# Createroner/InSAR-Unet-CA

Hardware: AMD Instinct MI355X
Metric: InSAR tiles/sec (fwd+bwd) U-Net-CA 256x256 (higher is better)
Workload: dtype bf16; 1 GPU; U-Net-CA (in=2, classes=2, use_se) bf16, batch 16x2x256x256 per GPU, Dice+CE + Adam(lr=1e-4) training on synthetic InSAR tiles; global_batch=16, parallelism=dp1

## Files before the change

### include/insar_hip.h

```cpp
#ifndef INSAR_HIP_H
#define INSAR_HIP_H

#include <stdint.h>

#ifdef __cplusplus
extern "C" {
#endif

#define INSAR_ABI_VERSION 8

enum { INSAR_F32 = 0, INSAR_BF16 = 1 };

enum {
  INSAR_OK = 0,
  INSAR_E_SHAPE = -1001,
  INSAR_E_DTYPE = -1002,
  INSAR_E_ALIGN = -1003,
  INSAR_E_WS = -1004,
  INSAR_E_ARG = -1005
};

typedef struct InsarAct {
  void* ptr;
  int32_t B, H, W;
// ... 27 lines not shown

typedef struct InsarIgemm {
  InsarAct x;
  InsarAct y;
  const void* w;
  const float* bias;
  float* stats;
  int32_t N;
  int32_t Ho, Wo;
  int32_t stride;
  int32_t ntaps;
  int32_t mode;
  int8_t dy[12], dx[12];
  int32_t flags;
  int32_t out_stride;
  int32_t out_oy, out_ox;
  int32_t _pad;
  const void* add;
  InsarBstat bstat;
  const void* gate;
} InsarIgemm;
enum { INSAR_IGEMM_OOB_ZERO = 1,
       INSAR_IGEMM_PINGPONG = 2  };
int insar_igemm_num_mtiles(int64_t M, int32_t N);
int insar_igemm_tile_rows(int64_t M, int32_t N);
int insar_igemm_tile_cols(int64_t M, int32_t N);
int insar_igemm_tile_cols_dt(int64_t M, int32_t N, int32_t dtype);
int insar_igemm(const InsarIgemm* d, void* stream);

int insar_conv3x3_flat_ok(const InsarAct* x, int32_t N);
int insar_conv3x3_flat_num_mtiles(const InsarAct* x);
int insar_conv3x3_flat_rows_ok(const InsarAct* x, int32_t N);
int insar_conv3x3_flat_rows_dil_ok(const InsarAct* x, int32_t N, int32_t dil);
int insar_conv3x3_flat2_rows_ok(const InsarAct* x, int32_t N);
int insar_conv3x3_flat_stat_rows(const InsarAct* x, int32_t N, int32_t flip);
int insar_conv3x3_flat(const InsarAct* x, const InsarAct* y, const void* w, int32_t flip, float* stats,
                       void* stream);
int insar_conv3x3_flat_bstat(const InsarAct* x, const InsarAct* y, const void* w, int32_t flip, float* stats,
                             const InsarBstat* bstat, void* stream);

int insar_conv3x3_c64_ok(const InsarAct* x, int32_t N);
int insar_conv3x3_c64_rows(const InsarAct* x);
int insar_conv3x3_c64_geometry(const InsarAct* x, int32_t* out);
int insar_conv3x3_c64(const InsarAct* x, const InsarAct* y, const void* w, int32_t flip, float* stats,
                      void* stream);
int insar_conv3x3_c64_bstat(const InsarAct* x, const InsarAct* y, const void* w, int32_t flip, float* stats,
                            const InsarBstat* bstat, void* stream);

typedef struct InsarWgrad {
  InsarAct x;
  InsarAct dy;
  const int32_t* tabx;
  const int32_t* tabdy;
  float* part;
  int64_t Mpad;
  int32_t nsplit;
  int32_t ntaps;
  int32_t offx[12];
  int32_t offdy[12];
  int64_t tabx_tap_stride;
} InsarWgrad;
int insar_wgrad_tile(int32_t C, int32_t dtype);
int insar_wgrad_tile_pair(int32_t Cin, int32_t Cout, int32_t dtype);
int insar_wgrad(const InsarWgrad* d, void* stream);
int insar_wgrad_conv3_tile(const InsarAct* x, int32_t Cout);
int insar_wgrad_conv3(const InsarAct* x, const InsarAct* dy, float* part, int32_t nsplit, void* stream);
int insar_wgrad_conv3x_tile(const InsarAct* x, int32_t Cout);
int insar_wgrad_conv3x(const InsarAct* x, const InsarAct* dy, float* part, int32_t nsplit, void* stream);
int insar_wgrad_conv3y_tile(const InsarAct* x, int32_t Cout);
int insar_wgrad_conv3y(const InsarAct* x, const InsarAct* dy, float* part, int32_t nsplit, void* stream);
int insar_wgrad_conv3k_tile(const InsarAct* x, int32_t Cout);
int insar_wgrad_conv3k_slices(const InsarAct* x, int32_t Cout);
int insar_wgrad_conv3k(const InsarAct* x, const InsarAct* dy, float* part, int32_t nsplit, void* stream);
int insar_wgrad_reduce(const float* part, float* grad, int32_t nsplit, int32_t ntaps, int32_t Co,
                       int32_t Ci, int32_t layout, int32_t accumulate, void* stream);
int insar_wgrad_fold(const float* part_in, float* part_out, int64_t slab_floats, int32_t nsplit,
                     int32_t group, void* stream);
int insar_pixel_table(int32_t* tab, int64_t Mpad, int32_t B, int32_t H, int32_t W, int32_t s,
                      int32_t Hb, int32_t Wb, int32_t tail, void* stream);

int insar_conv3x3_small_fwd_rows(const InsarAct* x, const InsarAct* y);
int insar_conv3x3_small_fwd(const InsarAct* x, const float* w ,
                            const InsarAct* y, float* stats , void* stream);
int insar_conv3x3_small_wgrad_blocks(int32_t B, int32_t H);
int insar_conv3x3_small_wgrad(const InsarAct* x, const InsarAct* dy, float* part, void* stream);
int insar_conv3x3_small_wgrad_fused_ok(const InsarAct* x, const InsarAct* y);
int insar_conv3x3_small_wgrad_fused(const InsarAct* x, const InsarAct* g, const InsarAct* y, const float* scale,
                                    const float* shift, const float* mean, const float* invstd, const float* k1,
                                    const float* k2, int32_t relu, float* part, void* stream);

int insar_colsum(const float* part, float* out, int32_t segments, int64_t rows, int32_t cols,
                 int32_t accumulate, float* tmp, int64_t tmp_floats, void* stream);
int insar_colsum_ld(const float* part, float* out, int32_t segments, int64_t rows, int32_t cols, int64_t ld,
                    int32_t accumulate, float* tmp, int64_t tmp_floats, void* stream);

int insar_colsum_partial(const float* part, float* out, int64_t rows, int32_t cols, int32_t rps,
                         void* stream);

typedef struct InsarBnFinalize {
  const float* part; int64_t rows; int64_t count; int32_t C; int32_t training;
  const float* conv_bias; const float* gamma; const float* beta;
  float* running_mean; float* running_var; int64_t* num_batches_tracked;
  float momentum; float eps;
  float* scale; float* shift; float* mean; float* invstd;
} InsarBnFinalize;
int insar_bn_finalize(const InsarBnFinalize* d, void* stream);
int insar_bn_relu_apply(const InsarAct* y, const float* scale, const float* shift,
                        const float* gate , const InsarAct* dst, int32_t relu,
                        void* stream);

int insar_bn_relu_apply_pool(const InsarAct* y, const float* scale, const float* shift, const float* gate,
                             const InsarAct* dst, const InsarAct* pooled, int32_t relu, void* stream);

int insar_se_squeeze(const InsarAct* y, const float* scale, const float* shift, float* part,
                     int32_t relu, int32_t rows_per_part, void* stream);
typedef struct InsarSeFwd {
  const float* part;
  int32_t B, H, W, C, Cr; int32_t rows;
  const float* scale; const float* shift;
  const float* w1;  const float* w2;
  float* pooled;
  float* sq; float* hid; float* gate;
} InsarSeFwd;
int insar_se_excite(const InsarSeFwd* d, void* stream);

int insar_bnrelu_bwd_reduce(const InsarAct* dout, const InsarAct* y, const float* scale,
                            const float* shift, float* part, int32_t relu, int32_t rows_per_part, void* stream);
typedef struct InsarBnSeBwd {
  int32_t B, H, W, C, Cr; int32_t use_se;
  const float* mean; const float* invstd;
  const float* pooled; const float* sq; const float* hid; const float* gate;
  const float* w1; const float* w2;
  float* dw1; float* dw2; float* dgamma; float* dbeta;
  float* coefB; float* k1; float* k2;
  int32_t accumulate; int32_t _pad;
} InsarBnSeBwd;
int insar_bnse_bwd_coef(const InsarBnSeBwd* d, const float* red, int32_t rows, const float* scale,
                        const float* shift, float* ws, float* dconv_bias, int32_t training, void* stream);
int insar_bnse_bwd_coef_fused(const InsarBnSeBwd* d, const float* red, int32_t rows, const float* scale,
                              const float* shift, float* ws, float* dconv_bias, int32_t training, uint32_t* ticket,
                              void* stream);
int insar_bn_bwd_coef(const InsarBnSeBwd* d, const float* red, int64_t rows_total, const float* scale,
                      float* dconv_bias, int32_t training, void* stream);
int insar_bnrelu_bwd_apply(const InsarAct* dout, const InsarAct* y, const float* scale,
                           const float* shift, const float* mean, const float* invstd,
                           const float* gate, const float* coefB, const float* k1,
                           const float* k2, const InsarAct* dy, int32_t relu, void* stream);
int insar_bnse_bwd_coef_stage(const InsarBnSeBwd* d, const float* red, int32_t rows, const float* scale,
                              const float* shift, float* ws, float* dconv_bias, int32_t training, int32_t stage,
                              void* stream);
int insar_bnrelu_bwd_apply_part(const InsarAct* dout, const InsarAct* y, const float* scale, const float* shift,
                                const float* mean, const float* invstd, const float* gate, const float* coefB,
                                const float* tb, const float* tg, const InsarAct* dy, int32_t relu, void* stream);

int insar_bn_relu_apply_pool_arg(const InsarAct* y, const float* scale, const float* shift, const float* gate,
                                 const InsarAct* dst, const InsarAct* pooled, uint8_t* arg, int32_t relu, void* stream);
int insar_bnrelu_bwd_reduce_pool(const InsarAct* dskip, const InsarAct* dpooled, const uint8_t* arg, const InsarAct* y,
                                 const float* scale, const float* shift, float* part, int32_t relu,
                                 int32_t rows_per_part, void* stream);
int insar_bnrelu_bwd_apply_pool(const InsarAct* dskip, const InsarAct* dpooled, const uint8_t* arg, const InsarAct* y,
                                const float* scale, const float* shift, const float* mean, const float* invstd,
                                const float* gate, const float* coefB, const float* k1, const float* k2,
                                const InsarAct* dy, int32_t relu, void* stream);

int insar_conv1x1_out_wgrad(const InsarAct* x, const float* w, const float* dlogits, int32_t K, float* part, void* stream);
int insar_bn_relu_apply_outc(const InsarAct* y, const float* scale, const float* shift, const float* gate ,
                             const float* wout, const float* bias , float* logits, int32_t K, int32_t relu,
                             void* stream);
int insar_conv1x1_out_wgrad_y(const InsarAct* y, const float* scale, const float* shift, const float* gate ,
                              const float* w, const float* dlogits, int32_t K, float* part, void* stream);
int insar_bnrelu_bwd_reduce_outc(const float* dlogits, const float* wout, int32_t K, const InsarAct* y,
                                 const float* scale, const float* shift, float* part, int32_t relu,
                                 int32_t rows_per_part, const float* gate, float* wpart, void* stream);
int insar_bnrelu_bwd_apply_outc(const float* dlogits, const float* wout, int32_t K, const InsarAct* y,
                                const float* scale, const float* shift, const float* mean, const float* invstd,
                                const float* gate, const float* coefB, const float* k1, const float* k2,
                                const InsarAct* dy, int32_t relu, void* stream);

typedef struct InsarCam {
  int32_t B, H, W, C, Cr; int32_t rows;
  const float* psum; const float* pmax; const int32_t* parg;
  const float* w1; const float* w2;
  float* avg; float* mx; int32_t* arg;
  float* ha; float* hm;
  float* gate;
  float* coefB; float* dmax;
  float* ws;
  float* dw1; float* dw2;
  int32_t accumulate; int32_t _pad;
} InsarCam;
int insar_cam_pool(const InsarAct* x, float* psum, float* pmax, int32_t* parg, int32_t rows_per_part,
                   void* stream);
int insar_cam_excite(const InsarCam* d, void* stream);
int insar_cam_bwd_coef(const InsarCam* d, const float* red , int32_t rows, void* stream);
int insar_cam_scatter_max(const InsarAct* dx, const float* dmax, const int32_t* arg, void* stream);

typedef struct InsarSa {
  InsarAct x;
  InsarAct y;
  float* comp;
  uint16_t* arg;
  float* z1; float* z2;
  float* s;
  float* g2; float* g1;
  float* dcomp;
  float* stat1; float* stat2;
  float* part;
  int32_t rows;
  int32_t training;
  const float* w1; const float* w2;
  const float* bn;
  float* coef;
  float* dw1; float* db1; float* dgamma1; float* dbeta1;
  float* dw2; float* db2; float* dgamma2; float* dbeta2;
} InsarSa;
int insar_sa_compress(const InsarSa* d, void* stream);
int insar_sa_conv(const InsarSa* d, int32_t which , void* stream);
int insar_sa_gate(const InsarSa* d, void* stream);
int insar_sa_dscale(const InsarSa* d, void* stream);
int insar_sa_bwd_coef(const InsarSa* d, int32_t stage , void* stream);
int insar_sa_bwd_stencil(const InsarSa* d, int32_t which , void* stream);
int insar_sa_dx(const InsarSa* d, void* stream);

int insar_maxpool2_fwd(const InsarAct* x, const InsarAct* y, void* stream);
int insar_maxpool2_bwd(const InsarAct* x, const InsarAct* dy, const InsarAct* dx, int32_t accumulate,
                       void* stream);

int insar_resize_bilinear_fwd(const InsarAct* src, const InsarAct* dst, void* stream);
int insar_resize_bilinear_bwd(const InsarAct* ddst, const InsarAct* dsrc, void* stream);

int insar_conv1x1_out_fwd(const InsarAct* x, const float* w , const float* bias,
                          float* logits , int32_t K, void* stream);
int insar_conv1x1_out_bwd_blocks(int32_t B, int32_t H);
int insar_conv1x1_out_bwd(const InsarAct* x, const float* w, const float* dlogits, int32_t K,
                          const InsarAct* dx, float* part, void* stream);

int insar_ce_blocks(int64_t npix);
int insar_cross_entropy(const float* logits, const int64_t* target, int32_t B, int32_t K, int64_t HW,
                        int64_t ignore_index, float* dlogits, float* loss_out, float* ws, void* stream);
int insar_dice(const float* logits, const int64_t* target, int32_t B, int32_t K, int64_t HW,
               int64_t ignore_index, float smooth, float* dlogits, float* loss_out, float* ws,
               void* stream);

int insar_dice_ce(const float* logits, const int64_t* target, int32_t B, int32_t K, int64_t HW,
                  int64_t ignore_index, float smooth, float ce_weight, float dice_weight, float* dlogits,
                  float* loss_out, float* ws, void* stream);

int insar_cross_entropy_w(const float* logits, const int64_t* target, int32_t B, int32_t K, int64_t HW,
                          int64_t ignore_index, const float* weight, float label_smoothing, float* dlogits,
                          float* loss_out, float* ws, void* stream);
int insar_focal(const float* logits, const int64_t* target, int32_t B, int32_t K, int64_t HW, int64_t ignore_index,
                float gamma, const float* alpha, float* dlogits, float* loss_out, float* ws, void* stream);
int insar_dice_ce_w(const float* logits, const int64_t* target, int32_t B, int32_t K, int64_t HW,
                    int64_t ignore_index, float smooth, float ce_weight, float dice_weight, const float* weight,
                    float label_smoothing, float focal_gamma, float* dlogits, float* loss_out, float* ws,
                    void* stream);
int insar_label_hist(const int64_t* target, int64_t npix, int32_t K, int64_t ignore_index, int64_t* counts,
                     int64_t* ws, void* stream);

int insar_confusion(const float* logits, const int64_t* target, int32_t B, int32_t K, int64_t HW,
                    int64_t ignore_index, int64_t* counts , void* stream);

enum { INSAR_SCENE_U8 = 0, INSAR_SCENE_F32 = 1 };
int insar_scene_gather(const void* scene, int32_t dtype , int32_t H, int32_t W, const int32_t* origins,
                       int32_t n, int32_t T, float* out , void* stream);
int insar_scene_blend(const float* logits, const int32_t* origins, int32_t n, int32_t K, int32_t T, int32_t overlap,
                      float* acc, float* wsum, int32_t H, int32_t W, int32_t y_lo, int32_t y_hi, int32_t x_lo, int32_t x_hi,
                      void* stream);
int insar_scene_finalize(const float* acc, const float* wsum, int32_t K, int32_t H, int32_t W, float* prob ,
                         uint8_t* mask, float* conf, void* stream);

typedef struct InsarRegion {
  int64_t area;
  int64_t sum_y, sum_x;
  int64_t sum_conf;
  int32_t y0, x0, y1, x1;
  int32_t root;
  int32_t cls;
  int32_t _pad[2];
} InsarRegion;
int insar_regions_scratch_bytes(int32_t H, int32_t W, int32_t max_regions, int64_t* scratch_bytes, int64_t* table_bytes);
int insar_regions_tiles(const uint8_t* mask, const float* conf , float min_conf, int32_t H, int32_t W,
                        int32_t connectivity, void* scratch, void* stream);
int insar_regions_merge(const uint8_t* mask, int32_t H, int32_t W, int32_t connectivity, void* scratch, void* stream);
int insar_regions_flatten(int32_t H, int32_t W, void* scratch, void* stream);
int insar_regions_number(const uint8_t* mask, int32_t H, int32_t W, int64_t min_area, int32_t max_regions, void* scratch,
                         void* table, void* stream);
int insar_regions_relabel(const uint8_t* mask, const float* conf , int32_t H, int32_t W, int32_t max_regions,
                          void* scratch, void* table, int32_t* labels, uint8_t* mask_out, void* stream);

typedef struct InsarOverlap {
  int32_t pred, gt;
  int64_t count;
} InsarOverlap;
int insar_overlap_scratch_bytes(int64_t max_pairs, int64_t* table_bytes, int64_t* out_bytes);
int insar_overlap_clear(void* table, void* out, int64_t max_pairs, void* stream);
int insar_overlap_count(const int32_t* pred, const int32_t* gt, const uint8_t* voidmap , int32_t void_value,
                        int32_t H, int32_t W, void* table, int64_t max_pairs, void* stream);
int insar_overlap_compact(const void* table, int64_t max_pairs, void* out, void* stream);

enum { INSAR_DIST_U8 = 0, INSAR_DIST_I32 = 1 };
enum { INSAR_DIST_EQ = 0, INSAR_DIST_NE = 1, INSAR_DIST_EDGE = 2 };
#define INSAR_DIST_FAR 0x7fffffff
int insar_dist_scratch_bytes(int32_t B, int32_t H, int32_t W, int64_t* scratch_bytes);
int insar_dist_transform(const void* m, int32_t elem_type, int32_t B, int32_t H, int32_t W, int32_t site_mode, int32_t value,
                         int32_t max_distance, void* scratch, int32_t* d2, int32_t* nearest , void* stream);
int insar_dist_boundary_counts(const uint8_t* pred, const uint8_t* gt, const int32_t* d2_pred, const int32_t* d2_gt, int32_t H,
                               int32_t W, int64_t r2, int32_t K, int32_t void_value, int64_t* counts, void* stream);

enum { INSAR_AUG_MASK_NONE = 0, INSAR_AUG_MASK_U8 = 1, INSAR_AUG_MASK_I64 = 2 };
int insar_aug_draw(uint64_t seed, uint64_t step, int32_t n, int32_t ops_mask, float gain_lo, float gain_hi, float bias_lo,
                   float bias_hi, float sigma_lo, float sigma_hi, int32_t* table, void* stream);
int insar_aug_apply(const float* x, float* xo, int32_t C, const void* m, int32_t m_dtype , int64_t* mo,
                    int32_t n, int32_t H, int32_t W, const int32_t* table, uint64_t noise_seed, void* stream);

int insar_crops_cells(const uint8_t* labels, int32_t H, int32_t W, int32_t K, int32_t g, int32_t* table, void* stream);
int insar_crops_sat(int32_t* table, int32_t K, int32_t Hc, int32_t Wc, void* stream);
int insar_crops_draw(uint64_t key, int32_t n, int32_t K, int32_t tries, const float* cum, int32_t min_count, int32_t max_void,
                     int32_t T, int32_t g, int32_t H, int32_t W, const int32_t* sat, int32_t* origins, int32_t* info, void* stream);
int insar_crops_gather(const void* scene, int32_t scene_dtype, const uint8_t* labels, int32_t H, int32_t W, const int32_t* origins,
                       int32_t n, int32_t T, float* images, void* masks, int32_t mask_dtype, void* stream);

int insar_adam_step(const int64_t* table, const int32_t* chunks, int32_t nchunks, int32_t chunk_elems,
                    float lr, float beta1, float beta2, float eps, float bias_correction1,
                    float bias_correction2_sqrt, float grad_scale, void* stream);

int insar_pixel_table_taps(int32_t* tab , int64_t Mpad, int32_t B, int32_t H, int32_t W, int32_t s,
                           int32_t Hb, int32_t Wb, int32_t ntaps, const int8_t* dy, const int8_t* dx, void* stream);
int insar_conv7x7s2_fwd_rows(int32_t B, int32_t H);
// ... 65 lines not shown
```

### insar_unet_ca_amd/_lib.py

```python
from __future__ import annotations

import ctypes as C
import os

import torch

_HERE = os.path.dirname(os.path.abspath(__file__))
LIB_PATH = os.environ.get("INSAR_HIP_LIB") or os.path.join(_HERE, "libinsar_hip.so")

F32, BF16 = 0, 1
ABI_VERSION = 8
SCENE_U8, SCENE_F32 = 0, 1
AUG_MASK_NONE, AUG_MASK_U8, AUG_MASK_I64 = 0, 1, 2
DIST_U8, DIST_I32 = 0, 1
DIST_EQ, DIST_NE, DIST_EDGE = 0, 1, 2
DIST_FAR = 0x7FFFFFFF
IGEMM_OOB_ZERO = 1
IGEMM_PINGPONG = 2


class InsarAct(C.Structure):
    _fields_ = [("ptr", C.c_void_p), ("B", C.c_int32), ("H", C.c_int32), ("W", C.c_int32),
                ("C", C.c_int32), ("c_off", C.c_int32), ("c_len", C.c_int32), ("dtype", C.c_int32),
                ("_pad", C.c_int32)]
# ... 41 lines not shown
                ("coefB", C.c_void_p), ("k1", C.c_void_p), ("k2", C.c_void_p),
                ("accumulate", C.c_int32), ("_pad", C.c_int32)]


class InsarCam(C.Structure):
    _fields_ = [("B", C.c_int32), ("H", C.c_int32), ("W", C.c_int32), ("C", C.c_int32), ("Cr", C.c_int32),
                ("rows", C.c_int32),
                ("psum", C.c_void_p), ("pmax", C.c_void_p), ("parg", C.c_void_p), ("w1", C.c_void_p), ("w2", C.c_void_p),
                ("avg", C.c_void_p), ("mx", C.c_void_p), ("arg", C.c_void_p), ("ha", C.c_void_p), ("hm", C.c_void_p),
                ("gate", C.c_void_p), ("coefB", C.c_void_p), ("dmax", C.c_void_p), ("ws", C.c_void_p),
                ("dw1", C.c_void_p), ("dw2", C.c_void_p), ("accumulate", C.c_int32), ("_pad", C.c_int32)]


class InsarSa(C.Structure):
    _fields_ = [("x", InsarAct), ("y", InsarAct), ("comp", C.c_void_p), ("arg", C.c_void_p),
                ("z1", C.c_void_p), ("z2", C.c_void_p), ("s", C.c_void_p), ("g2", C.c_void_p), ("g1", C.c_void_p),
                ("dcomp", C.c_void_p), ("stat1", C.c_void_p), ("stat2", C.c_void_p), ("part", C.c_void_p),
                ("rows", C.c_int32), ("training", C.c_int32), ("w1", C.c_void_p), ("w2", C.c_void_p),
                ("bn", C.c_void_p), ("coef", C.c_void_p),
                ("dw1", C.c_void_p), ("db1", C.c_void_p), ("dgamma1", C.c_void_p), ("dbeta1", C.c_void_p),
                ("dw2", C.c_void_p), ("db2", C.c_void_p), ("dgamma2", C.c_void_p), ("dbeta2", C.c_void_p)]


class InsarOptwState(C.Structure):
    _fields_ = [("t", C.c_int64), ("skipped", C.c_int64), ("bc1", C.c_float), ("bc2_sqrt", C.c_float), ("lr", C.c_float),
                ("coef", C.c_float), ("grad_norm", C.c_float), ("ema_alpha", C.c_float), ("skip", C.c_int32), ("_pad", C.c_int32)]


class InsarOptwConfig(C.Structure):
    _fields_ = [("lr", C.c_double), ("beta1", C.c_double), ("beta2", C.c_double), ("max_norm", C.c_double),
                ("warmup_start", C.c_double), ("min_lr", C.c_double), ("power", C.c_double), ("ema_decay", C.c_double),
                ("warmup_steps", C.c_int64), ("total_steps", C.c_int64), ("schedule", C.c_int32),
                ("skip_nonfinite", C.c_int32), ("ema_warmup", C.c_int32), ("_pad", C.c_int32)]


SCHED_NONE, SCHED_CONSTANT, SCHED_COSINE, SCHED_POLY = 0, 1, 2, 3

_P = C.c_void_p
_I = C.c_int32
_L = C.c_int64
_F = C.c_float
_AP = C.POINTER(InsarAct)

_SIGNATURES = {
    "insar_pack_nchw": [_P, _AP, _P],
    "insar_unpack_nchw": [_AP, _P, _P],
    "insar_weight_prep": [_P, _P, _I, _I, _I, _I, _L, _L, _L, _P],
    "insar_weight_prep_batch": [_P, _I, _L, _P],
    "insar_weight_prep_pair_batch": [_P, _I, _L, _P],
    "insar_igemm_num_mtiles": [_L, _I],
    "insar_igemm_tile_rows": [_L, _I],
    "insar_igemm_tile_cols": [_L, _I],
    "insar_igemm_tile_cols_dt": [_L, _I, _I],
    "insar_igemm": [C.POINTER(InsarIgemm), _P],
    "insar_conv3x3_flat_ok": [_AP, _I],
    "insar_conv3x3_flat_num_mtiles": [_AP],
    "insar_conv3x3_flat_rows_ok": [_AP, _I],
    "insar_conv3x3_flat2_rows_ok": [_AP, _I],
    "insar_conv3x3_flat_rows_dil_ok": [_AP, _I, _I],
    "insar_conv3x3_flat_stat_rows": [_AP, _I, _I],
    "insar_conv3x3_flat": [_AP, _AP, _P, _I, _P, _P],
    "insar_conv3x3_flat_bstat": [_AP, _AP, _P, _I, _P, C.POINTER(InsarBstat), _P],
    "insar_conv3x3_c64_ok": [_AP, _I],
    "insar_conv3x3_c64_rows": [_AP],
    "insar_conv3x3_c64_geometry": [_AP, _P],
    "insar_conv3x3_c64": [_AP, _AP, _P, _I, _P, _P],
    "insar_conv3x3_c64_bstat": [_AP, _AP, _P, _I, _P, C.POINTER(InsarBstat), _P],
    "insar_wgrad": [C.POINTER(InsarWgrad), _P],
    "insar_wgrad_tile": [_I, _I],
    "insar_wgrad_tile_pair": [_I, _I, _I],
    "insar_wgrad_conv3_tile": [_AP, _I],
    "insar_wgrad_conv3": [_AP, _AP, _P, _I, _P],
    "insar_wgrad_conv3x_tile": [_AP, _I],
    "insar_wgrad_conv3x": [_AP, _AP, _P, _I, _P],
    "insar_wgrad_conv3y_tile": [_AP, _I],
    "insar_wgrad_conv3y": [_AP, _AP, _P, _I, _P],
    "insar_wgrad_conv3k_tile": [_AP, _I],
    "insar_wgrad_conv3k_slices": [_AP, _I],
    "insar_wgrad_conv3k": [_AP, _AP, _P, _I, _P],
    "insar_wgrad_reduce": [_P, _P, _I, _I, _I, _I, _I, _I, _P],
    "insar_wgrad_fold": [_P, _P, _L, _I, _I, _P],
    "insar_pixel_table": [_P, _L, _I, _I, _I, _I, _I, _I, _I, _P],
    "insar_conv3x3_small_fwd": [_AP, _P, _AP, _P, _P],
    "insar_conv3x3_small_fwd_rows": [_AP, _AP],
    "insar_conv3x3_small_wgrad_blocks": [_I, _I],
    "insar_conv3x3_small_wgrad": [_AP, _AP, _P, _P],
    "insar_conv3x3_small_wgrad_fused_ok": [_P, _P],
    "insar_conv3x3_small_wgrad_fused": [_P, _P, _P, _P, _P, _P, _P, _P, _P, _I, _P, _P],
    "insar_colsum": [_P, _P, _I, _L, _I, _I, _P, _L, _P],
    "insar_colsum_ld": [_P, _P, _I, _L, _I, _L, _I, _P, _L, _P],
    "insar_colsum_partial": [_P, _P, _L, _I, _I, _P],
    "insar_bn_finalize": [C.POINTER(InsarBnFinalize), _P],
    "insar_bn_relu_apply": [_AP, _P, _P, _P, _AP, _I, _P],
    "insar_bn_relu_apply_pool": [_AP, _P, _P, _P, _AP, _AP, _I, _P],
    "insar_se_squeeze": [_AP, _P, _P, _P, _I, _I, _P],
    "insar_se_excite": [C.POINTER(InsarSeFwd), _P],
    "insar_bnrelu_bwd_reduce": [_AP, _AP, _P, _P, _P, _I, _I, _P],
    "insar_bnse_bwd_coef": [C.POINTER(InsarBnSeBwd), _P, _I, _P, _P, _P, _P, _I, _P],
    "insar_bnse_bwd_coef_fused": [C.POINTER(InsarBnSeBwd), _P, _I, _P, _P, _P, _P, _I, _P, _P],
    "insar_bn_bwd_coef": [C.POINTER(InsarBnSeBwd), _P, _L, _P, _P, _I, _P],
    "insar_bnrelu_bwd_apply": [_AP, _AP, _P, _P, _P, _P, _P, _P, _P, _P, _AP, _I, _P],
    "insar_bn_relu_apply_pool_arg": [_AP, _P, _P, _P, _AP, _AP, _P, _I, _P],
    "insar_bnrelu_bwd_reduce_pool": [_AP, _AP, _P, _AP, _P, _P, _P, _I, _I, _P],
    "insar_bnrelu_bwd_apply_pool": [_AP, _AP, _P, _AP, _P, _P, _P, _P, _P, _P, _P, _P, _AP, _I, _P],
    "insar_conv1x1_out_wgrad": [_AP, _P, _P, _I, _P, _P],
    "insar_bn_relu_apply_outc": [_AP, _P, _P, _P, _P, _P, _P, _I, _I, _P],
    "insar_conv1x1_out_wgrad_y": [_AP, _P, _P, _P, _P, _P, _I, _P, _P],
    "insar_bnrelu_bwd_reduce_outc": [_P, _P, _I, _AP, _P, _P, _P, _I, _I, _P, _P, _P],
    "insar_bnrelu_bwd_apply_outc": [_P, _P, _I, _AP, _P, _P, _P, _P, _P, _P, _P, _P, _AP, _I, _P],
    "insar_bnse_bwd_coef_stage": [C.POINTER(InsarBnSeBwd), _P, _I, _P, _P, _P, _P, _I, _I, _P],
    "insar_bnrelu_bwd_apply_part": [_AP, _AP, _P, _P, _P, _P, _P, _P, _P, _P, _AP, _I, _P],
    "insar_cam_pool": [_AP, _P, _P, _P, _I, _P],
    "insar_cam_excite": [C.POINTER(InsarCam), _P],
    "insar_cam_bwd_coef": [C.POINTER(InsarCam), _P, _I, _P],
    "insar_cam_scatter_max": [_AP, _P, _P, _P],
    "insar_sa_compress": [C.POINTER(InsarSa), _P],
    "insar_sa_conv": [C.POINTER(InsarSa), _I, _P],
    "insar_sa_gate": [C.POINTER(InsarSa), _P],
    "insar_sa_dscale": [C.POINTER(InsarSa), _P],
    "insar_sa_bwd_coef": [C.POINTER(InsarSa), _I, _P],
    "insar_sa_bwd_stencil": [C.POINTER(InsarSa), _I, _P],
    "insar_sa_dx": [C.POINTER(InsarSa), _P],
    "insar_resize_bilinear_fwd": [_AP, _AP, _P],
    "insar_resize_bilinear_bwd": [_AP, _AP, _P],
    "insar_maxpool2_fwd": [_AP, _AP, _P],
    "insar_maxpool2_bwd": [_AP, _AP, _AP, _I, _P],
    "insar_conv1x1_out_fwd": [_AP, _P, _P, _P, _I, _P],
    "insar_conv1x1_out_bwd_blocks": [_I, _I],
    "insar_conv1x1_out_bwd": [_AP, _P, _P, _I, _AP, _P, _P],
    "insar_ce_blocks": [_L],
    "insar_cross_entropy": [_P, _P, _I, _I, _L, _L, _P, _P, _P, _P],
    "insar_dice": [_P, _P, _I, _I, _L, _L, _F, _P, _P, _P, _P],
    "insar_dice_ce": [_P, _P, _I, _I, _L, _L, _F, _F, _F, _P, _P, _P, _P],
    "insar_confusion": [_P, _P, _I, _I, _L, _L, _P, _P],
    "insar_cross_entropy_w": [_P, _P, _I, _I, _L, _L, _P, _F, _P, _P, _P, _P],
    "insar_focal": [_P, _P, _I, _I, _L, _L, _F, _P, _P, _P, _P, _P],
    "insar_dice_ce_w": [_P, _P, _I, _I, _L, _L, _F, _F, _F, _P, _F, _F, _P, _P, _P, _P],
    "insar_label_hist": [_P, _L, _I, _L, _P, _P, _P],
    "insar_scene_gather": [_P, _I, _I, _I, _P, _I, _I, _P, _P],
    "insar_scene_blend": [_P, _P, _I, _I, _I, _I, _P, _P, _I, _I, _I, _I, _I, _I, _P],
    "insar_scene_finalize": [_P, _P, _I, _I, _I, _P, _P, _P, _P],
    "insar_regions_scratch_bytes": [_I, _I, _I, _P, _P],
    "insar_regions_tiles": [_P, _P, _F, _I, _I, _I, _P, _P],
    "insar_regions_merge": [_P, _I, _I, _I, _P, _P],
    "insar_regions_flatten": [_I, _I, _P, _P],
    "insar_regions_number": [_P, _I, _I, _L, _I, _P, _P, _P],
    "insar_regions_relabel": [_P, _P, _I, _I, _I, _P, _P, _P, _P, _P],
    "insar_overlap_scratch_bytes": [_L, _P, _P],
    "insar_overlap_clear": [_P, _P, _L, _P],
    "insar_overlap_count": [_P, _P, _P, _I, _I, _I, _P, _L, _P],
    "insar_overlap_compact": [_P, _L, _P, _P],
    "insar_dist_scratch_bytes": [_I, _I, _I, _P],
    "insar_dist_transform": [_P, _I, _I, _I, _I, _I, _I, _I, _P, _P, _P, _P],
    "insar_dist_boundary_counts": [_P, _P, _P, _P, _I, _I, _L, _I, _I, _P, _P],
    "insar_aug_draw": [C.c_uint64, C.c_uint64, _I, _I, _F, _F, _F, _F, _F, _F, _P, _P],
    "insar_aug_apply": [_P, _P, _I, _P, _I, _P, _I, _I, _I, _P, C.c_uint64, _P],
    "insar_crops_cells": [_P, _I, _I, _I, _I, _P, _P],
    "insar_crops_sat": [_P, _I, _I, _I, _P],
    "insar_crops_draw": [C.c_uint64, _I, _I, _I, _P, _I, _I, _I, _I, _I, _I, _P, _P, _P, _P],
    "insar_crops_gather": [_P, _I, _P, _I, _I, _P, _I, _I, _P, _P, _I, _P],
    "insar_adam_step": [_P, _P, _I, _I, _F, _F, _F, _F, _F, _F, _F, _P],
    "insar_scale_f32": [_P, _L, _F, _P],
    "insar_mul_dev_f32": [_P, _P, _L, _P, _P],
    "insar_adam_step_dev": [_P, _P, _I, _I, _F, C.c_double, C.c_double, _F, _P, _F, _P],
    "insar_gradnorm_partials": [_P, _P, _I, _I, _F, _P, _P],
    "insar_optw_advance": [_P, _P, _I, _P, _P],
    "insar_adamw_step": [_P, _P, _I, _I, _F, _F, _F, _F, _I, _P, _P],
    "insar_pixel_table_taps": [_P, _L, _I, _I, _I, _I, _I, _I, _I, _P, _P, _P],
    "insar_conv7x7s2_fwd_rows": [_I, _I],
    "insar_conv7x7s2_fwd": [_P, _I, _I, _P, _AP, _P, _P],
    "insar_conv7x7s2_wgrad_blocks": [_I, _I],
    "insar_conv7x7s2_wgrad": [_P, _I, _I, _AP, _P, _P],
    "insar_maxpool3s2_fwd": [_AP, _AP, _P, _P],
    "insar_maxpool3s2_bwd": [_AP, _P, _AP, _P],
    "insar_bn_add_relu": [_AP, _P, _P, _AP, _AP, _I, _P],
    "insar_relu_gate_bwd": [_AP, _AP, _AP, _P],
    "insar_se_res_apply": [_AP, _P, _P, _P, _AP, _AP, _P],
    "insar_sum_hw": [_AP, _AP, _F, _P],
    "insar_broadcast_hw": [_AP, _AP, _F, _I, _P],
    "insar_broadcast_hw_gate": [_AP, _AP, _AP, _F, _I, _P],
    "insar_dropout": [_AP, _AP, _P, C.c_uint64, _P, _F, _I, _P],
    "insar_bilinear_fwd": [_P, _P, _I, _I, _I, _I, _I, _P],
    "insar_bilinear_bwd": [_P, _P, _I, _I, _I, _I, _I, _P],
    "insar_tune_set": [C.c_char_p, _I],
    "insar_tune_get": [C.c_char_p],
}
EXPORTED_SYMBOLS = sorted(list(_SIGNATURES) + ["insar_version", "insar_last_error"])

_lib = None


class InsarError(RuntimeError):
    pass


def load():
    global _lib
    if _lib is not None:
        return _lib
    if not os.path.isfile(LIB_PATH):
        raise InsarError(
            f"{LIB_PATH} not found: build it with `python -c 'import __graft_entry__ as g; g.build()'` "
            "(there is no CPU / eager fallback for the HIP path)")
    lib = C.CDLL(LIB_PATH)
    lib.insar_version.restype = C.c_int
    lib.insar_version.argtypes = []
    lib.insar_last_error.restype = C.c_char_p
    lib.insar_last_error.argtypes = []
    for name, args in _SIGNATURES.items():
        fn = getattr(lib, name)
        fn.restype = C.c_int
        fn.argtypes = args
    if lib.insar_version() != ABI_VERSION:
        raise InsarError(f"libinsar_hip.so ABI {lib.insar_version()} != expected {ABI_VERSION}")
    _lib = lib
    for item in filter(None, os.environ.get("INSAR_TUNE", "").split(",")):
# ... 57 lines not shown
```

### insar_unet_ca_amd/csrc/direct.hip

```cpp
#include "common.h"

#define DR_THREADS 256
#define DR_MAXCI 4
#define DR_MAXK 8

template <typename T>
__device__ __forceinline__ float load_elem(const char* p) {
  if constexpr (sizeof(T) == 2) return bf16_to_f32(*(const uint16_t*)p);
  else return *(const float*)p;
}

template <typename T, int CI>
__device__ __forceinline__ void load_pixel(const char* p, float (&v)[CI]) {
  if constexpr (sizeof(T) == 2 && CI == 2) {
    const uint32_t u = *(const uint32_t*)p;
    v[0] = bf16_to_f32((uint16_t)(u & 0xffffu)); v[1] = bf16_to_f32((uint16_t)(u >> 16));
  } else if constexpr (sizeof(T) == 2 && CI == 4) {
    const uint2 u = *(const uint2*)p;
    v[0] = bf16_to_f32((uint16_t)(u.x & 0xffffu)); v[1] = bf16_to_f32((uint16_t)(u.x >> 16));
    v[2] = bf16_to_f32((uint16_t)(u.y & 0xffffu)); v[3] = bf16_to_f32((uint16_t)(u.y >> 16));
  } else if constexpr (sizeof(T) == 4 && CI == 2) {
    const float2 u = *(const float2*)p; v[0] = u.x; v[1] = u.y;
  } else if constexpr (sizeof(T) == 4 && CI == 4) {
    const float4 u = *(const float4*)p; v[0] = u.x; v[1] = u.y; v[2] = u.z; v[3] = u.w;
  } else {
#pragma unroll
    for (int ci = 0; ci < CI; ++ci) v[ci] = load_elem<T>(p + ci * sizeof(T));
  }
}

template <typename T, int CI>
__global__ void __launch_bounds__(DR_THREADS)
conv3x3_small_fwd_kernel(ActView x, const float* __restrict__ wt, ActView y, float* __restrict__ part) {
  constexpr int CH = Chunk<T>::N;
  __shared__ float red[DR_THREADS * (2 * CH + 1)];
  const int Co = y.c_len;
  const int cpp = Co / CH;
  const int rows = y.B * y.H;
  const int total = y.W * cpp;
  const int cc = threadIdx.x % cpp;
  typedef float f2 __attribute__((ext_vector_type(2)));
  f2 wr[9][CI][CH / 2];
#pragma unroll
  for (int tap = 0; tap < 9; ++tap)
#pragma unroll
    for (int ci = 0; ci < CI; ++ci)
#pragma unroll
      for (int j = 0; j < CH / 2; ++j) {
        wr[tap][ci][j].x = wt[((int64_t)(cc * CH + 2 * j) * CI + ci) * 9 + tap];
        wr[tap][ci][j].y = wt[((int64_t)(cc * CH + 2 * j + 1) * CI + ci) * 9 + tap];
      }
  for (int r = blockIdx.x; r < rows; r += gridDim.x) {
    const int n = r / y.H, h = r - n * y.H;
    float s1[CH], s2[CH];
#pragma unroll
    for (int j = 0; j < CH; ++j) { s1[j] = 0.f; s2[j] = 0.f; }
    for (int e = threadIdx.x; e < total; e += blockDim.x) {
      const int w = e / cpp;
      f2 acc2[CH / 2];
#pragma unroll
      for (int j = 0; j < CH / 2; ++j) acc2[j] = (f2){0.f, 0.f};
      const char* p0 = x.base + x.elem_offset(n, h - 1, w - 1) * (int64_t)sizeof(T);
#pragma unroll
      for (int tap = 0; tap < 9; ++tap) {
        float xv[CI];
        load_pixel<T, CI>(p0 + ((int64_t)(tap / 3) * (x.W + 2) + (tap % 3)) * x.C * (int64_t)sizeof(T), xv);
#pragma unroll
        for (int ci = 0; ci < CI; ++ci) {
          const f2 xx = (f2){xv[ci], xv[ci]};
#pragma unroll
          for (int j = 0; j < CH / 2; ++j) acc2[j] = __builtin_elementwise_fma(xx, wr[tap][ci][j], acc2[j]);
        }
      }
      float acc[CH];
#pragma unroll
      for (int j = 0; j < CH / 2; ++j) { acc[2 * j] = acc2[j].x; acc[2 * j + 1] = acc2[j].y; }
      const uint4 packed = Chunk<T>::pack(acc);
      float f[CH];
      Chunk<T>::unpack(packed, f);
#pragma unroll
      for (int j = 0; j < CH; ++j) { s1[j] += f[j]; s2[j] = fmaf(f[j], f[j], s2[j]); }
      *(uint4*)(y.base + (y.elem_offset(n, h, w) + (int64_t)cc * CH) * (int64_t)sizeof(T)) = packed;
    }
    if (part) {
#pragma unroll
      for (int j = 0; j < CH; ++j) { red[threadIdx.x * (2 * CH + 1) + j] = s1[j]; red[threadIdx.x * (2 * CH + 1) + CH + j] = s2[j]; }
      __syncthreads();
      for (int o = threadIdx.x; o < 2 * Co; o += blockDim.x) {
        const int q = o / Co, c = o - q * Co;
        const int occ = c / CH, j = c - occ * CH;
        float s = 0.f;
        for (int t = occ; t < blockDim.x; t += cpp) s += red[t * (2 * CH + 1) + q * CH + j];
        part[((int64_t)r * 2 + q) * Co + c] = s;
      }
      __syncthreads();
    }
  }
}

typedef __attribute__((ext_vector_type(8))) short d_bf16x8_t;
typedef __attribute__((ext_vector_type(4))) float d_f32x4_t;

template <int CI>
__global__ void __launch_bounds__(DR_THREADS) conv3x3_small_fwd_mfma_kernel(ActView x, const float* __restrict__ wt, ActView y,
                                                                           float* __restrict__ part) {
  constexpr int KV = 9 * CI;
  __shared__ float red[DR_THREADS / 64][2][64];
  const int lane = threadIdx.x & 63, wave = threadIdx.x >> 6, nw = blockDim.x >> 6;
  const int r16 = lane & 15, kq = lane >> 4;
  const int Co = y.c_len;
  d_bf16x8_t wf[4], wl[4];
#pragma unroll
  for (int nt = 0; nt < 4; ++nt)
#pragma unroll
    for (int i = 0; i < 8; ++i) {
      const int k = 8 * kq + i;
      float v = 0.f;
      if (k < KV) v = wt[((int64_t)(nt * 16 + r16) * CI + (k % CI)) * 9 + (k / CI)];
      const uint16_t hi = f32_to_bf16(v);
      wf[nt][i] = (short)hi;
      wl[nt][i] = (short)f32_to_bf16(v - bf16_to_f32(hi));
    }
  const int rows = y.B * y.H;
  const int groups = (y.W + 15) / 16;
  float s1[4][4], s2[4][4];
#pragma unroll
  for (int nt = 0; nt < 4; ++nt)
#pragma unroll
    for (int j = 0; j < 4; ++j) { s1[nt][j] = 0.f; s2[nt][j] = 0.f; }
  for (int r = blockIdx.x; r < rows; r += gridDim.x) {
    const int n = r / y.H, h = r - n * y.H;
    for (int g = wave; g < groups; g += nw) {
      const int w = g * 16 + r16;
      const bool ok = w < y.W;
      const int wc = ok ? w : y.W - 1;
      d_bf16x8_t xf;
      const char* p0 = x.base + x.elem_offset(n, h - 1, wc - 1) * (int64_t)sizeof(bf16_t);
      if constexpr (CI == 2) {
#pragma unroll
        for (int i = 0; i < 4; ++i) {
          const int tap = 4 * kq + i;
          uint32_t v = 0;
          if (tap < 9) v = *(const uint32_t*)(p0 + ((int64_t)(tap / 3) * (x.W + 2) + (tap % 3)) * x.C * 2);
          xf[2 * i] = (short)(v & 0xffffu); xf[2 * i + 1] = (short)(v >> 16);
        }
      } else {
#pragma unroll
        for (int i = 0; i < 8; ++i) {
          const int k = 8 * kq + i;
          short v = 0;
          if (k < KV) {
            const int tap = k / CI, ci = k - tap * CI;
            v = *(const short*)(p0 + (((int64_t)(tap / 3) * (x.W + 2) + (tap % 3)) * x.C + ci) * 2);
          }
          xf[i] = v;
        }
      }
      char* yp = y.base + (y.elem_offset(n, h, wc) + kq * 4) * (int64_t)2;
#pragma unroll
      for (int nt = 0; nt < 4; ++nt) {
        d_f32x4_t acc = (d_f32x4_t){0.f, 0.f, 0.f, 0.f};
        acc = __builtin_amdgcn_mfma_f32_16x16x32_bf16(wl[nt], xf, acc, 0, 0, 0);
        acc = __builtin_amdgcn_mfma_f32_16x16x32_bf16(wf[nt], xf, acc, 0, 0, 0);
        if (ok) {
          uint2 v;
          v.x = pack2_bf16(acc[0], acc[1]);
          v.y = pack2_bf16(acc[2], acc[3]);
          *(uint2*)(yp + nt * 32) = v;
          const float f0 = __uint_as_float(v.x << 16), f1 = __uint_as_float(v.x & 0xffff0000u);
          const float f2 = __uint_as_float(v.y << 16), f3 = __uint_as_float(v.y & 0xffff0000u);
          s1[nt][0] += f0; s2[nt][0] = fmaf(f0, f0, s2[nt][0]);
          s1[nt][1] += f1; s2[nt][1] = fmaf(f1, f1, s2[nt][1]);
          s1[nt][2] += f2; s2[nt][2] = fmaf(f2, f2, s2[nt][2]);
          s1[nt][3] += f3; s2[nt][3] = fmaf(f3, f3, s2[nt][3]);
        }
      }
    }
  }
  if (part) {
#pragma unroll
    for (int nt = 0; nt < 4; ++nt)
#pragma unroll
      for (int j = 0; j < 4; ++j) {
#pragma unroll
        for (int sh = 1; sh < 16; sh <<= 1) { s1[nt][j] += __shfl_xor(s1[nt][j], sh, 64); s2[nt][j] += __shfl_xor(s2[nt][j], sh, 64); }
        LDS_PIN(s1[nt][j]); LDS_PIN(s2[nt][j]);
      }
    if (r16 == 0) {
#pragma unroll
      for (int nt = 0; nt < 4; ++nt)
#pragma unroll
        for (int j = 0; j < 4; ++j) {
          red[wave][0][nt * 16 + kq * 4 + j] = s1[nt][j];
          red[wave][1][nt * 16 + kq * 4 + j] = s2[nt][j];
        }
    }
    LDS_DRAIN();
#pragma unroll
    for (int nt = 0; nt < 4; ++nt)
#pragma unroll
      for (int j = 0; j < 4; ++j) { LDS_KEEP(s1[nt][j]); LDS_KEEP(s2[nt][j]); }
    __syncthreads();
    if (threadIdx.x < 2 * Co) {
      const int q = threadIdx.x / Co, c = threadIdx.x - q * Co;
      float v = 0.f;
      for (int wv = 0; wv < nw; ++wv) v += red[wv][q][c];
      part[((int64_t)blockIdx.x * 2 + q) * Co + c] = v;
    }
  }
}

static int check_small(const InsarAct* x, const InsarAct* y, const char* who) {
  if (!x || !y || !x->ptr || !y->ptr) INSAR_FAIL(INSAR_E_ARG, "%s: null pointer", who);
  if (x->dtype != y->dtype) INSAR_FAIL(INSAR_E_DTYPE, "%s: dtype differ", who);
  if (x->B != y->B || x->H != y->H || x->W != y->W) INSAR_FAIL(INSAR_E_SHAPE, "%s: grid differs", who);
  if (x->c_len < 1 || x->c_len > DR_MAXCI) INSAR_FAIL(INSAR_E_SHAPE, "%s: Cin=%d must be 1..%d", who, x->c_len, DR_MAXCI);
  const int ch = y->dtype == INSAR_BF16 ? 8 : 4;
  const int cpp = y->c_len / ch;
  if (y->c_len % ch || cpp < 1 || cpp > 64 || (cpp & (cpp - 1)) || (DR_THREADS % cpp))
    INSAR_FAIL(INSAR_E_SHAPE, "%s: Cout=%d unsupported", who, y->c_len);
  return insar_check_act(y, who, "y");
}

static inline bool small_fwd_uses_mfma(const InsarAct* x, const InsarAct* y) {
  return y->dtype == INSAR_BF16 && y->c_len == 64 && x->c_len <= 3;
}
extern "C" int insar_conv3x3_small_fwd_rows(const InsarAct* x, const InsarAct* y) {
  if (!x || !y) return 0;
  const int64_t r = (int64_t)y->B * y->H;
  if (small_fwd_uses_mfma(x, y)) return (int)(r > 1024 ? 1024 : r);
  return (int)r;
}

extern "C" int insar_conv3x3_small_fwd(const InsarAct* x, const float* w, const InsarAct* y, float* stats, void* stream) {
  int rc;
  if ((rc = check_small(x, y, "insar_conv3x3_small_fwd"))) return rc;
  if (!w) INSAR_FAIL(INSAR_E_ARG, "insar_conv3x3_small_fwd: null weights");
  if ((x->c_len == 2 || x->c_len == 4) && (x->C % x->c_len || x->c_off % x->c_len))
    INSAR_FAIL(INSAR_E_SHAPE, "insar_conv3x3_small_fwd: input slice must be aligned to its %d channels", x->c_len);
  int grid = insar_grid_cap((int64_t)y->B * y->H);
  hipStream_t s = (hipStream_t)stream;
  const ActView xv = make_view(*x), yv = make_view(*y);
#define SMALL_FWD(T, CI) hipLaunchKernelGGL((conv3x3_small_fwd_kernel<T, CI>), dim3(grid), dim3(DR_THREADS), 0, s, xv, w, yv, stats)
  if (small_fwd_uses_mfma(x, y)) {
    grid = insar_conv3x3_small_fwd_rows(x, y);
    switch (x->c_len) {
      case 1: hipLaunchKernelGGL((conv3x3_small_fwd_mfma_kernel<1>), dim3(grid), dim3(DR_THREADS), 0, s, xv, w, yv, stats); break;
      case 2: hipLaunchKernelGGL((conv3x3_small_fwd_mfma_kernel<2>), dim3(grid), dim3(DR_THREADS), 0, s, xv, w, yv, stats); break;
      default: hipLaunchKernelGGL((conv3x3_small_fwd_mfma_kernel<3>), dim3(grid), dim3(DR_THREADS), 0, s, xv, w, yv, stats); break;
    }
  } else if (y->dtype == INSAR_BF16) {
    switch (x->c_len) { case 1: SMALL_FWD(bf16_t, 1); break; case 2: SMALL_FWD(bf16_t, 2); break;
                        case 3: SMALL_FWD(bf16_t, 3); break; default: SMALL_FWD(bf16_t, 4); break; }
  } else {
    switch (x->c_len) { case 1: SMALL_FWD(float, 1); break; case 2: SMALL_FWD(float, 2); break;
                        case 3: SMALL_FWD(float, 3); break; default: SMALL_FWD(float, 4); break; }
  }
#undef SMALL_FWD
  INSAR_CHECK_LAUNCH("insar_conv3x3_small_fwd");
  return INSAR_OK;
}

template <typename T, int CI> struct RawPixel;
template <> struct RawPixel<bf16_t, 2> {
  uint32_t u;
  __device__ __forceinline__ void load(const char* p) { u = *(const uint32_t*)p; }
  __device__ __forceinline__ void get(float (&v)[2]) const { v[0] = __uint_as_float(u << 16); v[1] = __uint_as_float(u & 0xffff0000u); }
};
template <> struct RawPixel<bf16_t, 1> {
  uint16_t u;
  __device__ __forceinline__ void load(const char* p) { u = *(const uint16_t*)p; }
  __device__ __forceinline__ void get(float (&v)[1]) const { v[0] = bf16_to_f32(u); }
};
template <int CI> struct RawPixel<float, CI> {
  float f[CI];
  __device__ __forceinline__ void load(const char* p) {
#pragma unroll
    for (int c = 0; c < CI; ++c) f[c] = *(const float*)(p + 4 * c);
  }
  __device__ __forceinline__ void get(float (&v)[CI]) const {
#pragma unroll
    for (int c = 0; c < CI; ++c) v[c] = f[c];
  }
};

template <typename T, int CIB>
__global__ void __launch_bounds__(DR_THREADS) conv3x3_small_wgrad_kernel(ActView x, ActView dy, float* __restrict__ part) {
  constexpr int CH = Chunk<T>::N;
  extern __shared__ float sm[];
  const int Ci = x.c_len, Co = dy.c_len;
  const int cpp = Co / CH;
  const int rows = dy.B * dy.H;
  const int total = dy.W * cpp;
  const int cc = threadIdx.x % cpp;
  const int lane = threadIdx.x & 63, wave = threadIdx.x >> 6;
  for (int ci0 = 0; ci0 < Ci; ci0 += CIB) {
    typedef float wf2 __attribute__((ext_vector_type(2)));
    wf2 acc2[CIB][9][CH / 2];
#pragma unroll
    for (int c = 0; c < CIB; ++c)
#pragma unroll
      for (int t = 0; t < 9; ++t)
#pragma unroll
        for (int j = 0; j < CH / 2; ++j) acc2[c][t][j] = (wf2){0.f, 0.f};
    const int64_t x_pix_bytes = (int64_t)x.C * (int64_t)sizeof(T), x_row_bytes = (int64_t)(x.W + 2) * x_pix_bytes;
    const int ipr = (total + blockDim.x - 1) / blockDim.x;
    const int nrow = (rows - (int)blockIdx.x + (int)gridDim.x - 1) / (int)gridDim.x;
    const int nit = nrow * ipr;
    uint4 gq = make_uint4(0u, 0u, 0u, 0u);
    RawPixel<T, CIB> xq[9];
    bool okq = false;
    auto fetch = [&](int k, int j) {
      const int r = blockIdx.x + k * gridDim.x, e0 = threadIdx.x + j * blockDim.x;
      okq = e0 < total;
      const int e = okq ? e0 : threadIdx.x % cpp;
      const int n = r / dy.H, h = r - n * dy.H, w = e / cpp;
      gq = *(const uint4*)(dy.base + (dy.elem_offset(n, h, w) + (int64_t)cc * CH) * (int64_t)sizeof(T));
      const char* xc = x.base + (x.elem_offset(n, h, w) + ci0) * (int64_t)sizeof(T);
#pragma unroll
      for (int t = 0; t < 9; ++t) xq[t].load(xc + (t / 3 - 1) * x_row_bytes + (t % 3 - 1) * x_pix_bytes);
    };
    int kq_ = 0, jq_ = 0;
    if (nit > 0) fetch(0, 0);
    for (int it = 0; it < nit; ++it) {
      const uint4 gv = gq;
      RawPixel<T, CIB> xr[9];
#pragma unroll
      for (int t = 0; t < 9; ++t) xr[t] = xq[t];
      const bool ok = okq;
      if (++jq_ == ipr) { jq_ = 0; ++kq_; }
      fetch(it + 1 < nit ? kq_ : 0, it + 1 < nit ? jq_ : 0);
      float g[CH];
      Chunk<T>::unpack(gv, g);
      wf2 g2[CH / 2];
#pragma unroll
      for (int j = 0; j < CH / 2; ++j) g2[j] = ok ? (wf2){g[2 * j], g[2 * j + 1]} : (wf2){0.f, 0.f};
#pragma unroll
      for (int t = 0; t < 9; ++t) {
        float xv[CIB];
        xr[t].get(xv);
#pragma unroll
        for (int c = 0; c < CIB; ++c) {
// ... 671 lines not shown
```

### insar_unet_ca_amd/csrc/loss_optim.hip

```cpp
#include "common.h"

#define LO_THREADS 256
#define LO_MAXBLOCKS 1024
#define LO_MAXK 16

extern "C" int insar_ce_blocks(int64_t npix) {
  int64_t b = (npix + LO_THREADS - 1) / LO_THREADS;
  if (b < 1) b = 1;
  return (int)(b > LO_MAXBLOCKS ? LO_MAXBLOCKS : b);
}

__device__ __forceinline__ float block_sum(float v, float* red) {
  v = wave_sum(v);
  const int lane = threadIdx.x & 63, wave = threadIdx.x >> 6;
  __syncthreads();
  if (lane == 0) red[wave] = v;
  __syncthreads();
  float s = 0.f;
  for (int w = 0; w < (int)(blockDim.x >> 6); ++w) s += red[w];
  return s;
}

__global__ void ce_count_kernel(const int64_t* __restrict__ target, int64_t npix, int64_t ignore_index, float* ws) {
  __shared__ float red[8];
// ... 224 lines not shown
      if (q < stride) {
        const float c = block_sum(((v[0][q] + v[1][q]) + v[2][q]) + v[3][q], red);
        if (threadIdx.x == 0) tot[q] = c;
      }
    }
  } else {
    for (int q = 0; q < stride; ++q) {
      float c = 0.f;
      for (int i = threadIdx.x; i < nb; i += blockDim.x) c += ws[3 + 3 * K + (int64_t)i * stride + q];
      c = block_sum(c, red);
      if (threadIdx.x == 0) tot[q] = c;
    }
  }
  __syncthreads();
  if (threadIdx.x == 0) {
    const float nvalid = tot[0];
    ws[0] = nvalid; ws[1] = 1.f / nvalid; ws[2] = tot[1];
    float acc = 0.f;
    for (int k = 0; k < K; ++k) {
      ws[3 + k] = tot[2 + k]; ws[3 + K + k] = tot[2 + K + k]; ws[3 + 2 * K + k] = tot[2 + 2 * K + k];
      acc += (2.f * tot[2 + k] + smooth) / (tot[2 + K + k] + tot[2 + 2 * K + k] + smooth);
    }
    const float ce = tot[1] / nvalid, dice = 1.f - acc / (float)K;
    loss_out[0] = ce_w * ce + dice_w * dice;
    loss_out[1] = ce;
    loss_out[2] = dice;
  }
}

template <int KT>
__global__ void dicece_partial_v4(const float* __restrict__ logits, const int64_t* __restrict__ target, int64_t HW,
                                  int64_t npix, int64_t ignore_index, float* ws) {
  __shared__ float red[8];
  float aI[KT], aP[KT], aT[KT];
  float cnt = 0.f, lsum = 0.f;
#pragma unroll
  for (int k = 0; k < KT; ++k) { aI[k] = 0.f; aP[k] = 0.f; aT[k] = 0.f; }
  const int64_t ngroups = npix >> 2;
  for (int64_t gi = blockIdx.x * (int64_t)blockDim.x + threadIdx.x; gi < ngroups; gi += (int64_t)gridDim.x * blockDim.x) {
    const int64_t p = gi << 2;
    const int64_t n = p / HW, hw = p - n * HW;
    const longlong2 t01 = *(const longlong2*)(target + p), t23 = *(const longlong2*)(target + p + 2);
    float4 lv[KT];
#pragma unroll
    for (int k = 0; k < KT; ++k) lv[k] = *(const float4*)(logits + (n * KT + k) * HW + hw);
    const int64_t tt[4] = {t01.x, t01.y, t23.x, t23.y};
#pragma unroll
    for (int e = 0; e < 4; ++e) {
      const int64_t t = tt[e];
      if (t == ignore_index) continue;
      float v[KT];
#pragma unroll
      for (int k = 0; k < KT; ++k) v[k] = ((const float*)&lv[k])[e];
      float mx = v[0];
#pragma unroll
      for (int k = 1; k < KT; ++k) mx = fmaxf(mx, v[k]);
      float se = 0.f;
#pragma unroll
      for (int k = 0; k < KT; ++k) se += __expf(v[k] - mx);
      const float rse = 1.f / se;
      const float lse = mx + __logf(se);
      cnt += 1.f;
#pragma unroll
      for (int k = 0; k < KT; ++k) {
        const float pr = __expf(v[k] - mx) * rse;
        aP[k] += pr;
        if (k == t) { aI[k] += pr; aT[k] += 1.f; lsum += lse - v[k]; }
      }
    }
  }
  float* out = ws + 3 + 3 * KT + (int64_t)blockIdx.x * (2 + 3 * KT);
  const float c = block_sum(cnt, red), l = block_sum(lsum, red);
  if (threadIdx.x == 0) { out[0] = c; out[1] = l; }
#pragma unroll
  for (int k = 0; k < KT; ++k) {
    const float i = block_sum(aI[k], red), pp = block_sum(aP[k], red), tt = block_sum(aT[k], red);
    if (threadIdx.x == 0) { out[2 + k] = i; out[2 + KT + k] = pp; out[2 + 2 * KT + k] = tt; }
  }
}

template <int KT>
__global__ void dicece_grad_v4(const float* __restrict__ logits, const int64_t* __restrict__ target, int64_t HW,
                               int64_t npix, int64_t ignore_index, float smooth, float ce_w, float dice_w,
                               const float* __restrict__ ws, float* __restrict__ dlogits) {
  float num[KT], den[KT];
  const float inv = ws[1] * ce_w;
#pragma unroll
  for (int k = 0; k < KT; ++k) {
    num[k] = 2.f * ws[3 + k] + smooth;
    den[k] = ws[3 + KT + k] + ws[3 + 2 * KT + k] + smooth;
  }
  const int64_t ngroups = npix >> 2;
  for (int64_t gi = blockIdx.x * (int64_t)blockDim.x + threadIdx.x; gi < ngroups; gi += (int64_t)gridDim.x * blockDim.x) {
    const int64_t p = gi << 2;
    const int64_t n = p / HW, hw = p - n * HW;
    const longlong2 t01 = *(const longlong2*)(target + p), t23 = *(const longlong2*)(target + p + 2);
    float4 lv[KT], gv[KT];
#pragma unroll
    for (int k = 0; k < KT; ++k) lv[k] = *(const float4*)(logits + (n * KT + k) * HW + hw);
    const int64_t tt[4] = {t01.x, t01.y, t23.x, t23.y};
#pragma unroll
    for (int e = 0; e < 4; ++e) {
      const int64_t t = tt[e];
      float v[KT], o[KT];
#pragma unroll
      for (int k = 0; k < KT; ++k) { v[k] = ((const float*)&lv[k])[e]; o[k] = 0.f; }
      if (t != ignore_index) {
        float mx = v[0];
#pragma unroll
        for (int k = 1; k < KT; ++k) mx = fmaxf(mx, v[k]);
        float se = 0.f;
#pragma unroll
        for (int k = 0; k < KT; ++k) se += __expf(v[k] - mx);
        const float rse = 1.f / se;
        float pr[KT], gk[KT];
        float dot = 0.f;
#pragma unroll
        for (int k = 0; k < KT; ++k) {
          pr[k] = __expf(v[k] - mx) * rse;
          gk[k] = -((k == t ? 2.f * den[k] : 0.f) - num[k]) / (den[k] * den[k]) / (float)KT;
          dot = fmaf(pr[k], gk[k], dot);
        }
#pragma unroll
        for (int k = 0; k < KT; ++k) o[k] = (pr[k] - (k == t ? 1.f : 0.f)) * inv + dice_w * pr[k] * (gk[k] - dot);
      }
#pragma unroll
      for (int k = 0; k < KT; ++k) ((float*)&gv[k])[e] = o[k];
    }
#pragma unroll
    for (int k = 0; k < KT; ++k) *(float4*)(dlogits + (n * KT + k) * HW + hw) = gv[k];
  }
}

__global__ void dicece_grad_kernel(const float* __restrict__ logits, const int64_t* __restrict__ target, int K, int64_t HW,
                                   int64_t npix, int64_t ignore_index, float smooth, float ce_w, float dice_w,
                                   const float* __restrict__ ws, float* __restrict__ dlogits) {
  float num[LO_MAXK], den[LO_MAXK];
  const float inv = ws[1] * ce_w;
#pragma unroll
  for (int k = 0; k < LO_MAXK; ++k) {
    num[k] = k < K ? 2.f * ws[3 + k] + smooth : 0.f;
    den[k] = k < K ? ws[3 + K + k] + ws[3 + 2 * K + k] + smooth : 1.f;
  }
  for (int64_t p = blockIdx.x * (int64_t)blockDim.x + threadIdx.x; p < npix; p += (int64_t)gridDim.x * blockDim.x) {
    const int64_t n = p / HW, hw = p - n * HW;
    const float* lp = logits + n * K * HW + hw;
    float* gp = dlogits + n * K * HW + hw;
    const int64_t t = target[p];
    if (t == ignore_index) { for (int k = 0; k < K; ++k) gp[k * HW] = 0.f; continue; }
    float mx = lp[0];
    for (int k = 1; k < K; ++k) mx = fmaxf(mx, lp[k * HW]);
    float se = 0.f;
    for (int k = 0; k < K; ++k) se += __expf(lp[k * HW] - mx);
    const float rse = 1.f / se;
    float pr[LO_MAXK], gk[LO_MAXK];
    float dot = 0.f;
#pragma unroll
    for (int k = 0; k < LO_MAXK; ++k) {
      if (k < K) {
        pr[k] = __expf(lp[k * HW] - mx) * rse;
        gk[k] = -((k == t ? 2.f * den[k] : 0.f) - num[k]) / (den[k] * den[k]) / (float)K;
        dot = fmaf(pr[k], gk[k], dot);
      }
    }
#pragma unroll
    for (int k = 0; k < LO_MAXK; ++k)
      if (k < K) gp[k * HW] = (pr[k] - (k == t ? 1.f : 0.f)) * inv + dice_w * pr[k] * (gk[k] - dot);
  }
}

extern "C" int insar_dice_ce(const float* logits, const int64_t* target, int32_t B, int32_t K, int64_t HW, int64_t ignore_index,
                             float smooth, float ce_weight, float dice_weight, float* dlogits, float* loss_out, float* ws,
                             void* stream) {
  if (!logits || !target || !dlogits || !loss_out || !ws) INSAR_FAIL(INSAR_E_ARG, "insar_dice_ce: null pointer");
  if (K < 1 || K > LO_MAXK) INSAR_FAIL(INSAR_E_SHAPE, "insar_dice_ce: num_classes=%d must be 1..%d", K, LO_MAXK);
  if (B < 1 || HW < 1) INSAR_FAIL(INSAR_E_SHAPE, "insar_dice_ce: bad shape");
  const int64_t npix = (int64_t)B * HW;
  const int nb = insar_ce_blocks(npix);
  hipStream_t s = (hipStream_t)stream;
  const bool v4 = K >= 2 && K <= 4 && (HW & 3) == 0 && insar_aligned16(logits) && insar_aligned16(target) && insar_aligned16(dlogits);
#define DICECE_V4(KT)                                                                                                              \
  do {                                                                                                                             \
    hipLaunchKernelGGL(dicece_partial_v4<KT>, dim3(nb), dim3(LO_THREADS), 0, s, logits, target, HW, npix, ignore_index, ws);        \
    hipLaunchKernelGGL(dicece_final_kernel, dim3(1), dim3(LO_THREADS), 0, s, ws, K, nb, smooth, ce_weight, dice_weight, loss_out); \
    hipLaunchKernelGGL(dicece_grad_v4<KT>, dim3(nb), dim3(LO_THREADS), 0, s, logits, target, HW, npix, ignore_index, smooth,        \
                       ce_weight, dice_weight, ws, dlogits);                                                                        \
  } while (0)
  if (v4 && K == 2) DICECE_V4(2);
  else if (v4 && K == 3) DICECE_V4(3);
  else if (v4 && K == 4) DICECE_V4(4);
  else {
    hipLaunchKernelGGL(dicece_partial_kernel, dim3(nb), dim3(LO_THREADS), 0, s, logits, target, K, HW, npix, ignore_index, ws);
    hipLaunchKernelGGL(dicece_final_kernel, dim3(1), dim3(LO_THREADS), 0, s, ws, K, nb, smooth, ce_weight, dice_weight, loss_out);
    hipLaunchKernelGGL(dicece_grad_kernel, dim3(nb), dim3(LO_THREADS), 0, s, logits, target, K, HW, npix, ignore_index, smooth,
                       ce_weight, dice_weight, ws, dlogits);
  }
#undef DICECE_V4
  INSAR_CHECK_LAUNCH("insar_dice_ce");
  return INSAR_OK;
}

__global__ void confusion_kernel(const float* __restrict__ logits, const int64_t* __restrict__ target, int K, int64_t HW,
                                 int64_t npix, int64_t ignore_index, unsigned long long* counts) {
  extern __shared__ unsigned int sc[];
  for (int i = threadIdx.x; i < 3 * K; i += blockDim.x) sc[i] = 0;
  __syncthreads();
  for (int64_t p = blockIdx.x * (int64_t)blockDim.x + threadIdx.x; p < npix; p += (int64_t)gridDim.x * blockDim.x) {
    const int64_t t = target[p];
    if (t == ignore_index) continue;
    const int64_t n = p / HW, hw = p - n * HW;
    const float* lp = logits + n * K * HW + hw;
    int best = 0; float mx = lp[0];
    for (int k = 1; k < K; ++k) { const float v = lp[k * HW]; if (v > mx) { mx = v; best = k; } }
    if (best == (int)t) atomicAdd(&sc[best], 1u);
    else {
      atomicAdd(&sc[K + best], 1u);
      if (t >= 0 && t < K) atomicAdd(&sc[2 * K + (int)t], 1u);
    }
  }
  __syncthreads();
  for (int i = threadIdx.x; i < 3 * K; i += blockDim.x)
    if (sc[i]) atomicAdd(&counts[i], (unsigned long long)sc[i]);
}

extern "C" int insar_confusion(const float* logits, const int64_t* target, int32_t B, int32_t K, int64_t HW,
                               int64_t ignore_index, int64_t* counts, void* stream) {
  if (!logits || !target || !counts) INSAR_FAIL(INSAR_E_ARG, "insar_confusion: null pointer");
  if (K < 1 || K > 1024) INSAR_FAIL(INSAR_E_SHAPE, "insar_confusion: bad num_classes");
  const int64_t npix = (int64_t)B * HW;
  hipStream_t s = (hipStream_t)stream;
  hipError_t e = hipMemsetAsync(counts, 0, (size_t)3 * K * sizeof(int64_t), s);
  if (e != hipSuccess) INSAR_FAIL(-(int)e, "insar_confusion: memset: %s", hipGetErrorString(e));
  const int nb = insar_ce_blocks(npix);
  hipLaunchKernelGGL(confusion_kernel, dim3(nb), dim3(LO_THREADS), (size_t)3 * K * sizeof(unsigned int), s, logits, target, K, HW,
                     npix, ignore_index, (unsigned long long*)counts);
  INSAR_CHECK_LAUNCH("insar_confusion");
  return INSAR_OK;
}

template <bool DEV>
__global__ void adam_kernel(const int64_t* __restrict__ table, const int32_t* __restrict__ chunks, int chunk_elems,
                            float lr_over_bc1, float b1, float b2, float eps, float inv_bc2_sqrt, float gscale,
                            const float* __restrict__ state) {
  if constexpr (DEV) {
    lr_over_bc1 = lr_over_bc1 / state[1];
    inv_bc2_sqrt = 1.f / state[2];
  }
  const int ti = chunks[2 * blockIdx.x], ci = chunks[2 * blockIdx.x + 1];
  float* p = (float*)table[5 * ti + 0];
  const float* g = (const float*)table[5 * ti + 1];
  float* m = (float*)table[5 * ti + 2];
  float* v = (float*)table[5 * ti + 3];
  const int64_t numel = table[5 * ti + 4];
  const int64_t beg = (int64_t)ci * chunk_elems;
  int64_t end = beg + chunk_elems; if (end > numel) end = numel;
  const bool vec = (((uintptr_t)p | (uintptr_t)g | (uintptr_t)m | (uintptr_t)v) & 15) == 0;
  const float omb1 = 1.f - b1, omb2 = 1.f - b2;
  if (vec) {
    const int64_t end4 = beg + ((end - beg) & ~(int64_t)3);
    for (int64_t i = beg + threadIdx.x * 4; i < end4; i += (int64_t)blockDim.x * 4) {
      float4 pp = *(float4*)(p + i), gg = *(const float4*)(g + i), mm = *(float4*)(m + i), vv = *(float4*)(v + i);
      float* pa = (float*)&pp; float* ga = (float*)&gg; float* ma = (float*)&mm; float* va = (float*)&vv;
#pragma unroll
      for (int j = 0; j < 4; ++j) {
        const float gj = ga[j] * gscale;
        ma[j] = ma[j] + (gj - ma[j]) * omb1;
        va[j] = va[j] * b2 + omb2 * gj * gj;
        pa[j] = pa[j] - lr_over_bc1 * (ma[j] / (sqrtf(va[j]) * inv_bc2_sqrt + eps));
      }
      *(float4*)(p + i) = pp; *(float4*)(m + i) = mm; *(float4*)(v + i) = vv;
    }
    for (int64_t i = end4 + threadIdx.x; i < end; i += blockDim.x) {
      const float gj = g[i] * gscale;
      const float mj = m[i] + (gj - m[i]) * omb1;
      const float vj = v[i] * b2 + omb2 * gj * gj;
      m[i] = mj; v[i] = vj;
      p[i] = p[i] - lr_over_bc1 * (mj / (sqrtf(vj) * inv_bc2_sqrt + eps));
    }
  } else {
    for (int64_t i = beg + threadIdx.x; i < end; i += blockDim.x) {
      const float gj = g[i] * gscale;
// ... 37 lines not shown
```

### insar_unet_ca_amd/csrc/pointwise.hip

```cpp
#include "common.h"

#define PW_THREADS 256

struct RowIter {
  int n, h;
};

template <typename T>
__device__ __forceinline__ const uint4* chunk_ptr(const ActView& v, int n, int h, int w, int cc) {
  return (const uint4*)(v.base + (v.elem_offset(n, h, w) + (int64_t)cc * Chunk<T>::N) * (int64_t)sizeof(T));
}
template <typename T>
__device__ __forceinline__ uint4* chunk_ptr_w(const ActView& v, int n, int h, int w, int cc) {
  return (uint4*)(v.base + (v.elem_offset(n, h, w) + (int64_t)cc * Chunk<T>::N) * (int64_t)sizeof(T));
}

template <typename T>
__global__ void pack_scalar_kernel(const float* __restrict__ src, ActView dst, int Csrc) {
  const int64_t HW = (int64_t)dst.H * dst.W;
  const int64_t total = (int64_t)dst.B * HW;
  for (int64_t p = blockIdx.x * (int64_t)blockDim.x + threadIdx.x; p < total; p += (int64_t)gridDim.x * blockDim.x) {
    int n = (int)(p / HW);
    int64_t rem = p - (int64_t)n * HW;
    int h = (int)(rem / dst.W), w = (int)(rem - (int64_t)h * dst.W);
// ... 832 lines not shown
            const T* py = (const T*)(y.base + (y.elem_offset(n, h, w) + c) * (int64_t)sizeof(T));
            float f, gg = 1.f;
            if constexpr (sizeof(T) == 2) f = bf16_to_f32(*(const uint16_t*)py); else f = *(const float*)py;
            if constexpr (WITH_G) {
              const T* pg = (const T*)(g.base + (g.elem_offset(n, h, w) + c) * (int64_t)sizeof(T));
              if constexpr (sizeof(T) == 2) gg = bf16_to_f32(*(const uint16_t*)pg); else gg = *(const float*)pg;
            }
            const float m = (!relu || fmaf(f, sc, sh) > 0.f) ? gg : 0.f;
            s0 += m; s1 = fmaf(m, f, s1);
          }
        part[((int64_t)r * 2 + 0) * y.c_len + c] = s0;
        part[((int64_t)r * 2 + 1) * y.c_len + c] = s1;
      }
    }
  }
}

extern "C" int insar_se_squeeze(const InsarAct* y, const float* scale, const float* shift, float* part, int32_t relu,
                                int32_t rows_per_part, void* stream) {
  int rc;
  if ((rc = insar_check_act(y, "insar_se_squeeze", "y"))) return rc;
  if (!scale || !shift || !part) INSAR_FAIL(INSAR_E_ARG, "insar_se_squeeze: null pointer");
  if (rows_per_part < 1) INSAR_FAIL(INSAR_E_SHAPE, "insar_se_squeeze: rows_per_part");
  const int rpp = rows_per_part;
  int grid = insar_grid_cap((int64_t)y->B * ((y->H + rpp - 1) / rpp));
  hipStream_t s = (hipStream_t)stream;
  ActView v = make_view(*y);
  if (y->dtype == INSAR_BF16) hipLaunchKernelGGL((row_reduce_kernel<bf16_t, false>), dim3(grid), dim3(PW_THREADS), 0, s, v, v, scale, shift, part, relu, rpp, OutcGrad{nullptr, nullptr, 0, nullptr, nullptr}, PoolGrad{ActView{}, nullptr});
  else hipLaunchKernelGGL((row_reduce_kernel<float, false>), dim3(grid), dim3(PW_THREADS), 0, s, v, v, scale, shift, part, relu, rpp, OutcGrad{nullptr, nullptr, 0, nullptr, nullptr}, PoolGrad{ActView{}, nullptr});
  INSAR_CHECK_LAUNCH("insar_se_squeeze");
  return INSAR_OK;
}

static int check_outc_grad(const InsarAct* y, const float* dlogits, const float* wout, int32_t K, const char* who) {
  if (!dlogits || !wout) INSAR_FAIL(INSAR_E_ARG, "%s: null dlogits / weight", who);
  if (K < 1 || K > OG_MAXK) INSAR_FAIL(INSAR_E_SHAPE, "%s: num_classes=%d must be 1..%d", who, K, OG_MAXK);
  const int ch = y->dtype == INSAR_BF16 ? 8 : 4;
  if (y->c_len % ch || PW_THREADS % (y->c_len / ch)) INSAR_FAIL(INSAR_E_SHAPE, "%s: C=%d unsupported", who, y->c_len);
  return INSAR_OK;
}

static int check_pool_grad(const InsarAct* y, const InsarAct* dp, const uint8_t* arg, const char* who) {
  int rc;
  if (!dp || !arg) INSAR_FAIL(INSAR_E_ARG, "%s: null pooled gradient / arg-max map", who);
  if ((rc = insar_check_act(dp, who, "dpooled"))) return rc;
  if ((y->H & 1) || (y->W & 1) || dp->B != y->B || dp->H != y->H / 2 || dp->W != y->W / 2 || dp->c_len != y->c_len || dp->dtype != y->dtype)
    INSAR_FAIL(INSAR_E_SHAPE, "%s: pooled gradient must be (B, H/2, W/2, C) of an even grid", who);
  const int ch = y->dtype == INSAR_BF16 ? 8 : 4;
  if (y->c_len % ch || PW_THREADS % (y->c_len / ch)) INSAR_FAIL(INSAR_E_SHAPE, "%s: C=%d unsupported", who, y->c_len);
  return INSAR_OK;
}

static int launch_bwd_reduce(const char* who, const InsarAct* dout, const InsarAct* y, const float* scale, const float* shift,
                             float* part, int32_t relu, int32_t rows_per_part, OutcGrad og, PoolGrad pg, void* stream) {
  int rc;
  if ((rc = insar_check_act(y, who, "y"))) return rc;
  if (!og.dl) {
    if ((rc = insar_check_act(dout, who, "dout"))) return rc;
    if ((rc = check_same_grid(y, dout, who))) return rc;
  }
  if (!scale || !shift || !part) INSAR_FAIL(INSAR_E_ARG, "%s: null pointer", who);
  if (rows_per_part < 1) INSAR_FAIL(INSAR_E_SHAPE, "%s: rows_per_part", who);
  const int rpp = rows_per_part;
  int grid = insar_grid_cap((int64_t)y->B * ((y->H + rpp - 1) / rpp));
  hipStream_t s = (hipStream_t)stream;
  const ActView vy = make_view(*y), vg = og.dl ? vy : make_view(*dout);
  if (og.dl && og.K <= 2) {
    if (y->dtype == INSAR_BF16) hipLaunchKernelGGL((row_reduce_kernel<bf16_t, true, 2>), dim3(grid), dim3(PW_THREADS), 0, s, vg, vy, scale, shift, part, relu, rpp, og, pg);
    else hipLaunchKernelGGL((row_reduce_kernel<float, true, 2>), dim3(grid), dim3(PW_THREADS), 0, s, vg, vy, scale, shift, part, relu, rpp, og, pg);
  } else if (og.dl) {
    if (y->dtype == INSAR_BF16) hipLaunchKernelGGL((row_reduce_kernel<bf16_t, true, OG_MAXK>), dim3(grid), dim3(PW_THREADS), 0, s, vg, vy, scale, shift, part, relu, rpp, og, pg);
    else hipLaunchKernelGGL((row_reduce_kernel<float, true, OG_MAXK>), dim3(grid), dim3(PW_THREADS), 0, s, vg, vy, scale, shift, part, relu, rpp, og, pg);
  } else if (pg.arg) {
    if (y->dtype == INSAR_BF16) hipLaunchKernelGGL((row_reduce_kernel<bf16_t, true, 0, true>), dim3(grid), dim3(PW_THREADS), 0, s, vg, vy, scale, shift, part, relu, rpp, og, pg);
    else hipLaunchKernelGGL((row_reduce_kernel<float, true, 0, true>), dim3(grid), dim3(PW_THREADS), 0, s, vg, vy, scale, shift, part, relu, rpp, og, pg);
  } else {
    if (y->dtype == INSAR_BF16) hipLaunchKernelGGL((row_reduce_kernel<bf16_t, true>), dim3(grid), dim3(PW_THREADS), 0, s, vg, vy, scale, shift, part, relu, rpp, og, pg);
    else hipLaunchKernelGGL((row_reduce_kernel<float, true>), dim3(grid), dim3(PW_THREADS), 0, s, vg, vy, scale, shift, part, relu, rpp, og, pg);
  }
  INSAR_CHECK_LAUNCH(who);
  return INSAR_OK;
}

extern "C" int insar_bnrelu_bwd_reduce(const InsarAct* dout, const InsarAct* y, const float* scale, const float* shift,
                                       float* part, int32_t relu, int32_t rows_per_part, void* stream) {
  return launch_bwd_reduce("insar_bnrelu_bwd_reduce", dout, y, scale, shift, part, relu, rows_per_part,
                           OutcGrad{nullptr, nullptr, 0, nullptr, nullptr}, PoolGrad{ActView{}, nullptr}, stream);
}

extern "C" int insar_bnrelu_bwd_reduce_pool(const InsarAct* dskip, const InsarAct* dpooled, const uint8_t* arg, const InsarAct* y,
                                            const float* scale, const float* shift, float* part, int32_t relu,
                                            int32_t rows_per_part, void* stream) {
  int rc;
  if ((rc = insar_check_act(y, "insar_bnrelu_bwd_reduce_pool", "y"))) return rc;
  if ((rc = check_pool_grad(y, dpooled, arg, "insar_bnrelu_bwd_reduce_pool"))) return rc;
  return launch_bwd_reduce("insar_bnrelu_bwd_reduce_pool", dskip, y, scale, shift, part, relu, rows_per_part,
                           OutcGrad{nullptr, nullptr, 0, nullptr, nullptr}, PoolGrad{make_view(*dpooled), arg}, stream);
}

extern "C" int insar_bnrelu_bwd_reduce_outc(const float* dlogits, const float* wout, int32_t K, const InsarAct* y,
                                            const float* scale, const float* shift, float* part, int32_t relu,
                                            int32_t rows_per_part, const float* gate, float* wpart, void* stream) {
  int rc;
  if ((rc = insar_check_act(y, "insar_bnrelu_bwd_reduce_outc", "y"))) return rc;
  if ((rc = check_outc_grad(y, dlogits, wout, K, "insar_bnrelu_bwd_reduce_outc"))) return rc;
  return launch_bwd_reduce("insar_bnrelu_bwd_reduce_outc", nullptr, y, scale, shift, part, relu, rows_per_part,
                           OutcGrad{dlogits, wout, K, gate, wpart}, PoolGrad{ActView{}, nullptr}, stream);
}

#define COEF_THREADS 1024

__device__ __forceinline__ float strided_sum16(const float* __restrict__ p, int first, int rows, int step, int64_t ld) {
  float a[16];
#pragma unroll
  for (int u = 0; u < 16; ++u) a[u] = 0.f;
  int r = first;
  for (; r + 15 * step < rows; r += 16 * step) {
    float v[16];
#pragma unroll
    for (int u = 0; u < 16; ++u) v[u] = p[(int64_t)(r + u * step) * ld];
#pragma unroll
    for (int u = 0; u < 16; ++u) a[u] += v[u];
  }
  if (r + 7 * step < rows) {
    float v[8];
#pragma unroll
    for (int u = 0; u < 8; ++u) v[u] = p[(int64_t)(r + u * step) * ld];
#pragma unroll
    for (int u = 0; u < 8; ++u) a[u] += v[u];
    r += 8 * step;
  }
  if (r + 3 * step < rows) {
    float v[4];
#pragma unroll
    for (int u = 0; u < 4; ++u) v[u] = p[(int64_t)(r + u * step) * ld];
#pragma unroll
    for (int u = 0; u < 4; ++u) a[u] += v[u];
    r += 4 * step;
  }
  for (; r < rows; r += step) a[0] += p[(int64_t)r * ld];
  return (((a[0] + a[1]) + (a[2] + a[3])) + ((a[4] + a[5]) + (a[6] + a[7]))) +
         (((a[8] + a[9]) + (a[10] + a[11])) + ((a[12] + a[13]) + (a[14] + a[15])));
}

__device__ __forceinline__ void block_colsum(const float* __restrict__ slab, int rows, int cols, float* out, float* scratch) {
  const int nt = blockDim.x;
  if (cols >= nt) {
    for (int c = threadIdx.x; c < cols; c += nt) out[c] = strided_sum16(slab + c, 0, rows, 1, cols);
    __syncthreads();
  } else {
    const int lanes = nt / cols;
    const int c = threadIdx.x % cols, rl = threadIdx.x / cols;
    scratch[threadIdx.x] = rl < lanes ? strided_sum16(slab + c, rl, rows, lanes, cols) : 0.f;
    __syncthreads();
    if (threadIdx.x < cols) {
      float t = 0.f;
      for (int l = 0; l < lanes; ++l) t += scratch[l * cols + threadIdx.x];
      out[threadIdx.x] = t;
    }
    __syncthreads();
  }
}

__global__ void __launch_bounds__(COEF_THREADS) se_excite_kernel(InsarSeFwd d) {
  extern __shared__ float sm[];
  float* sq = sm;
  float* hid = sm + d.C;
  float* pool = hid + d.Cr;
// ... 853 lines not shown
```

### insar_unet_ca_amd/engine.py

```python
from __future__ import annotations

import contextlib
import ctypes as C
import os
from typing import Dict, List, Optional

import torch

from . import _lib, tape
from ._lib import InsarAct, InsarBnFinalize, InsarBnSeBwd, InsarIgemm, InsarSa, InsarSeFwd, InsarWgrad, call, ptr
from .tape import tape_py

BN_ROW_PIX = 128
WG_BKP = 64


def _round_up(a: int, b: int) -> int:
    return (a + b - 1) // b * b


class Act:

    def __init__(self, buf: torch.Tensor, B: int, H: int, W: int, Ctot: int, c_off: int, c_len: int):
        self.buf, self.B, self.H, self.W, self.C, self.c_off, self.c_len = buf, B, H, W, Ctot, c_off, c_len
# ... 193 lines not shown
            self._key[which] = self.key()
        return self._buf[which]

    def fwd(self) -> torch.Tensor:
        return self._get("fwd")

    def dgrad(self) -> torch.Tensor:
        return self._get("dgrad")


class WeightSet:

    def __init__(self, ctx: Ctx, weights: List[GemmWeight]):
        self.ctx, self.weights = ctx, weights
        self._jobs = None
        self._ptrs = None
        self._total = 0
        self._by_stage = None

    def stage_sets(self, groups) -> List["WeightSet"]:
        if self._by_stage is None:
            owner = {id(p): i for i, g in enumerate(groups) for p in g}
            buckets = [[] for _ in groups]
            for w in self.weights:
                buckets[owner[id(w.param)]].append(w)
            self._by_stage = [WeightSet(self.ctx, b) if b else None for b in buckets]
        return self._by_stage

    def stale(self) -> bool:
        return any(w._key["fwd"] != w.key() or w._key["dgrad"] != w.key() for w in self.weights)

    def refresh(self) -> None:
        tape.tape_live(self._refresh_now)

    def _refresh_now(self) -> None:
        if not self.stale():
            return
        ptrs = tuple(w.param.data_ptr() for w in self.weights)
        if self._jobs is None or ptrs != self._ptrs:
            rows, tile0 = [], 0
            for w in self.weights:
                a, b = w.param.shape[0], w.param.shape[1]
                T = w.param.shape[2] * w.param.shape[3]
                oab, oba = (w._buf["fwd"], w._buf["dgrad"]) if w.kind == "conv3" else (w._buf["dgrad"], w._buf["fwd"])
                rows.append([w.master().data_ptr(), oab.data_ptr(), oba.data_ptr(), a, b, T, tile0, w.ctx.code])
                tile0 += ((a + 31) // 32) * ((b + 31) // 32)
            self._jobs = torch.tensor(rows, dtype=torch.int64).to(self.ctx.device)
            self._ptrs, self._total = ptrs, tile0
        call("insar_weight_prep_pair_batch", ptr(self._jobs), self._jobs.shape[0], self._total, _lib.stream_ptr())
        for w in self.weights:
            w._key["fwd"] = w._key["dgrad"] = w.key()


class KernelTimer:

    def __init__(self, alone: bool = True):
        self.alone = alone
        self.elapsed = 0.0
        self.records: Dict[str, list] = {}

    def run(self, tag: str, flops: float, fn, nbytes: float = 0.0) -> None:
        e0, e1 = torch.cuda.Event(enable_timing=True), torch.cuda.Event(enable_timing=True)
        e0.record()
        fn()
        e1.record()
        self.records.setdefault(tag, []).append((e0, e1, flops, nbytes))

    def summary(self) -> Dict[str, dict]:
        torch.cuda.synchronize()
        out = {}
        for tag, recs in self.records.items():
            ms = sum(r[0].elapsed_time(r[1]) for r in recs)
            fl = sum(r[2] for r in recs)
            out[tag] = {"launches": len(recs), "ms": ms, "flops": fl, "bytes": sum(r[3] for r in recs),
                        "avg_us": 1e3 * ms / max(len(recs), 1), "tflops": fl / (ms * 1e-3) / 1e12 if ms > 0 else 0.0}
        return out


PROFILER: Optional[KernelTimer] = None
SPLIT_COEF = os.environ.get("INSAR_SPLIT_COEF", "0") == "1"
POOL_FUSE = os.environ.get("INSAR_POOL_FUSE", "1") != "0"
SMALL_WGRAD_FUSE = os.environ.get("INSAR_SMALL_WGRAD_FUSE", "1") != "0"
SMALL_WGRAD_MAIN = os.environ.get("INSAR_SMALL_WGRAD_MAIN", "1") != "0"
PREP_SIDE = os.environ.get("INSAR_PREP_SIDE", "1") != "0"
OUTC_FUSE = os.environ.get("INSAR_OUTC_FUSE", "1") != "0"
WGRAD_GRID_CAP = int(os.environ.get("INSAR_WGRAD_GRID_CAP", "200"))
COEF_FUSE = os.environ.get("INSAR_COEF_FUSE", "1") != "0"
COEF_SIMPLE = os.environ.get("INSAR_COEF_SIMPLE", "1") != "0"
OUTC_WGRAD_FUSE = os.environ.get("INSAR_OUTC_WGRAD_FUSE", "1") != "0"
WGRAD_FILL_T = float(os.environ.get("INSAR_WGRAD_FILL_T", "0.7"))
WGRAD_FILL_DL = float(os.environ.get("INSAR_WGRAD_FILL_DL", "0.5"))
WGRAD_FILL_ALONE = float(os.environ.get("INSAR_WGRAD_FILL_ALONE", "1.0"))
WGRAD_FILL_SMALL = float(os.environ.get("INSAR_WGRAD_FILL_SMALL", os.environ.get("INSAR_WGRAD_FILL", "0.5")))
WGRAD_FILL = float(os.environ.get("INSAR_WGRAD_FILL", "0.5"))
WGRAD_ROWS = os.environ.get("INSAR_WGRAD_ROWS", "1") != "0"
WGRAD_K = os.environ.get("INSAR_WGRAD_K", "0") != "0"
WGRAD_K_TILES = set(os.environ.get("INSAR_WGRAD_K_TILES", "128x64,128x128").split(","))
WGRAD_X = os.environ.get("INSAR_WGRAD_X", "1") != "0"
WGRAD_Y = int(os.environ.get("INSAR_WGRAD_Y", "0"))
FLAT_PP = int(os.environ.get("INSAR_FLAT_PP", "1"))
FLAT_PERSIST = int(os.environ.get("INSAR_FLAT_PERSIST", "2"))
IGEMM_PP = int(os.environ.get("INSAR_IGEMM_PP", "1"))
STAT_PREFOLD_ROWS = int(os.environ.get("INSAR_STAT_PREFOLD_ROWS", "1024"))
FLAT_ROWS = os.environ.get("INSAR_FLAT_ROWS", "1") != "0"
FLAT2 = int(os.environ.get("INSAR_FLAT2", "1"))
FLAT2_PERSIST = int(os.environ.get("INSAR_FLAT2_PERSIST", "1"))
FLAT2_KMAX = int(os.environ.get("INSAR_FLAT2_KMAX", "512"))
BSTAT_FUSE = os.environ.get("INSAR_BSTAT_FUSE", "1") != "0"
BSTAT_C64 = os.environ.get("INSAR_BSTAT_C64", "1") != "0"
WGRAD_LATE = os.environ.get("INSAR_WGRAD_ORDER", "before") == "after"


_TAPS3 = [(r - 1, s - 1) for r in range(3) for s in range(3)]
_TAPS3_DGRAD = [(1 - r, 1 - s) for r in range(3) for s in range(3)]
_TAPS2 = [(a, b) for a in range(2) for b in range(2)]


def _launch(tag, flops, fn, nbytes=0.0) -> None:
    if PROFILER is None:
        fn()
        return
    tag, flops, nbytes = (v() if callable(v) else v for v in (tag, flops, nbytes))
    PROFILER.run(tag, flops, fn, nbytes)


def _igemm(x: Act, y: Act, w, N: int, Ho: int, Wo: int, stride: int, taps, mode: int,
           bias: Optional[torch.Tensor] = None, stats: Optional[torch.Tensor] = None, oob: bool = False,
           add: Optional[Act] = None, out_stride: int = 1, out_off=(0, 0), bstat=None, gate: Optional[Act] = None) -> None:
    d = InsarIgemm()
    if bstat is not None:
        d.bstat.y, d.bstat.scale, d.bstat.shift = bstat[0].buf.data_ptr(), ptr(bstat[1]), ptr(bstat[2])
    d.x, d.y = x.desc, y.desc
    d.w, d.bias, d.stats = (w if isinstance(w, int) else ptr(w)), ptr(bias), ptr(stats)
    d.N, d.Ho, d.Wo, d.stride, d.ntaps, d.mode = N, Ho, Wo, stride, len(taps), mode
    d.flags = (_lib.IGEMM_OOB_ZERO if oob else 0) | (_lib.IGEMM_PINGPONG if IGEMM_PP else 0)
    d.out_stride, d.out_oy, d.out_ox = out_stride, out_off[0], out_off[1]
    if add is not None:
        if add.C != y.C or add.c_off != y.c_off or add.buf.dtype != y.buf.dtype or add.buf.shape != y.buf.shape:
            raise _lib.InsarError("igemm: `add` must have the output's buffer layout")
        d.add = add.buf.data_ptr()
    if gate is not None:
        if gate.C != y.C or gate.c_off != y.c_off or gate.buf.dtype != y.buf.dtype or gate.buf.shape != y.buf.shape:
            raise _lib.InsarError("igemm: `gate` must have the output's buffer layout")
        d.gate = gate.buf.data_ptr()
    for i, (dy, dx) in enumerate(taps):
        d.dy[i], d.dx[i] = dy, dx
    if PROFILER is not None:
        flops = 2.0 * x.B * Ho * Wo * N * x.c_len * len(taps)
        bm = call("insar_igemm_tile_rows", x.B * Ho * Wo, N)
        bn = call("insar_igemm_tile_cols_dt", x.B * Ho * Wo, N, x.code)
        if oob and x.code == _lib.F32:
            bn = 64
        tag = "igemm_kernel<%s, %d, %d, %d%s>%s" % ("float" if x.code == _lib.F32 else "bf16_t", bm, bn,
                                                    3 if bm == 256 and bn < 256 else 2, ", oob" if oob else "",
                                                    " +bstat" if bstat is not None else "")
        es = 2 if x.code == _lib.BF16 else 4
        nbytes = es * (x.B * x.H * x.W * x.c_len + y.B * y.H * y.W * y.c_len + len(taps) * N * x.c_len)
        PROFILER.run(tag, flops, lambda: call("insar_igemm", C.byref(d), _lib.stream_ptr()), nbytes)
        return
    call("insar_igemm", C.byref(d), _lib.stream_ptr())


def _flat_persist(flip: int) -> bool:
    return FLAT_PERSIST == 2 or (FLAT_PERSIST == 1 and not (flip & 1))


# ... 116 lines not shown

    def __init__(self, ctx: Ctx, params, groups: Optional[List[List[torch.nn.Parameter]]] = None):
        if groups is None:
            groups = [list(params)]
        self.params = [p for g in groups for p in g]
        self.groups = [list(g) for g in groups]
        offs, self.group_sizes, total = flat_layout(groups)
        self.flats = [torch.zeros(total, dtype=torch.float32, device=ctx.device) for _ in range(2)]
        self.views = [{id(p): f[o:o + p.numel()].view(p.shape) for p, o in zip(self.params, offs)} for f in self.flats]
        self.active = 0

    def select(self) -> None:
        for which in (0, 1):
            base, n = self.flats[which].data_ptr(), self.flats[which].numel() * 4
            if not any(p.grad is not None and base <= p.grad.data_ptr() < base + n for p in self.params):
                self.active = which
                return
        self.active = 0

    def view(self, p: torch.nn.Parameter) -> torch.Tensor:
        return self.views[self.active][id(p)]

    def flat(self) -> torch.Tensor:
        return self.flats[self.active]


def double_conv_params(mod) -> List[torch.nn.Parameter]:
    seq = mod.double_conv
    ps = [seq[0].weight, seq[0].bias, seq[1].weight, seq[1].bias,
          seq[3].weight, seq[3].bias, seq[4].weight, seq[4].bias]
    if len(seq) > 6:
        ps += [seq[6].fc[0].weight, seq[6].fc[2].weight]
    return ps


def grad_groups(net) -> List[List[torch.nn.Parameter]]:
    ups = [net.up1, net.up2, net.up3, net.up4]
    convs = [net.conv1, net.conv2, net.conv3, net.conv4]
    encs = [net.inc, net.down1[1], net.down2[1], net.down3[1], net.down4[1]]
    sas = [getattr(net, f"sa{i + 1}") for i in range(4)] if getattr(net, "spatial_attention", False) else None
    sa = lambda i: double_conv_params(sas[i].compress_and_map) if sas else []
    groups = [[net.outc.weight, net.outc.bias] + double_conv_params(convs[3]) + sa(3) + [ups[3].weight, ups[3].bias]]
    for i in (2, 1, 0):
        groups.append(double_conv_params(convs[i]) + sa(i) + [ups[i].weight, ups[i].bias])
    for l in (4, 3, 2, 1, 0):
        groups.append(double_conv_params(encs[l]))
    return groups


def bn_finalize_desc(bn, part: int, rows: int, count: int, C: int, training: bool, conv_bias: int,
                     scale: int, shift: int, mean: int, invstd: int) -> InsarBnFinalize:
    d = InsarBnFinalize()
    d.part, d.rows, d.count, d.C, d.training = part, rows, count, C, int(training)
    d.conv_bias = conv_bias
    d.gamma, d.beta = ptr(bn.weight), ptr(bn.bias)
    d.running_mean, d.running_var = ptr(bn.running_mean), ptr(bn.running_var)
    d.num_batches_tracked = ptr(bn.num_batches_tracked)
    d.momentum = bn.momentum if bn.momentum is not None else 0.1
    d.eps = bn.eps
    d.scale, d.shift, d.mean, d.invstd = scale, shift, mean, invstd
    return d


def bn_bwd_desc(B: int, H: int, W: int, C: int, bn, sink: "GradSink", mean, invstd, k1, k2) -> InsarBnSeBwd:
    d = InsarBnSeBwd()
    d.B, d.H, d.W, d.C, d.Cr, d.use_se = B, H, W, C, 1, 0
    d.mean, d.invstd = ptr(mean), ptr(invstd)
    d.dgamma, d.dbeta = ptr(sink.view(bn.weight)), ptr(sink.view(bn.bias))
    d.k1, d.k2 = ptr(k1), ptr(k2)
    d.accumulate = 0
    return d


class ConvBN:

    def __init__(self, ctx: Ctx, conv: torch.nn.Conv2d, bn: torch.nn.BatchNorm2d, x: Act, name: str):
        self.ctx, self.conv, self.bn, self.x, self.name = ctx, conv, bn, x, name
        B, H, W = x.B, x.H, x.W
        self.cin, self.cout = conv.in_channels, conv.out_channels
        if x.c_len != self.cin:
            raise _lib.InsarError(f"{name}: input slice has {x.c_len} channels, conv expects {self.cin}")
        self.small = self.cin <= 4
        self._small_part = None
        if not self.small and self.cin % 64:
            raise _lib.InsarError(f"{name}: in_channels={self.cin} must be <=4 or a multiple of 64 on the HIP path")
        if self.cout % 64:
            raise _lib.InsarError(f"{name}: out_channels={self.cout} must be a multiple of 64 on the HIP path")
        self.M = B * H * W
        self.y = Act.alloc(B, H, W, self.cout, ctx.dtype, ctx.device)
        c64_mode = os.environ.get("INSAR_C64", "1")
        self.c64 = (not self.small) and bool(call("insar_conv3x3_c64_ok", x.ref, self.cout)) and c64_mode != "0"
        self.c64_fwd, self.c64_bwd = self.c64 and c64_mode != "bwd", self.c64 and c64_mode != "fwd"
        self.flat_fwd = (not self.small) and not self.c64 and bool(call("insar_conv3x3_flat_ok", x.ref, self.cout))
        self.flat_bwd = (not self.small) and not self.c64 and bool(call("insar_conv3x3_flat_ok", x.ref, self.cin))
        plain = not (self.small or self.c64)
        self.rows_fwd = _rows_flags(x, self.cout) if (plain and not self.flat_fwd) else 0
        self.rows_bwd = _rows_flags(x, self.cin, self.cout, flip=1) if (plain and not self.flat_bwd) else 0
        if self.small:
            self.stat_rows = call("insar_conv3x3_small_fwd_rows", x.ref, self.y.ref)
        elif self.rows_fwd:
            self.stat_rows = call("insar_conv3x3_flat_stat_rows", x.ref, self.cout, self.rows_fwd)
        elif self.c64_fwd:
            self.stat_rows = call("insar_conv3x3_c64_rows", x.ref)
        elif self.c64:
            self.stat_rows = call("insar_igemm_num_mtiles", self.M, self.cout)
        elif self.flat_fwd:
            self.stat_rows = call("insar_conv3x3_flat_stat_rows", x.ref, self.cout, _flat_flags(0, x))
        else:
            self.stat_rows = call("insar_igemm_num_mtiles", self.M, self.cout)
        self.stats = ctx.f32(self.stat_rows, 2, self.cout)
        self.stat_rps = 0 if self.stat_rows <= STAT_PREFOLD_ROWS else max(64, -(-self.stat_rows // 64))
        self.fold_rows = self.stat_rows if not self.stat_rps else -(-self.stat_rows // self.stat_rps)
        self.sums = ctx.f32(self.fold_rows, 2, self.cout) if self.stat_rps else self.stats
        self.scale, self.shift = ctx.f32(self.cout), ctx.f32(self.cout)
        self.mean, self.invstd = ctx.f32(self.cout), ctx.f32(self.cout)
        self.k12 = ctx.f32(2, self.cout)
        self.k1, self.k2 = self.k12[0], self.k12[1]
        self._ticket = None
        self.sync_sums = None
        self.sync = None
        self.red_rpp = _rows_per_part(B, H)
        self.red_rows = -(-H // self.red_rpp)
        self.red_part = ctx.f32(B * self.red_rows, 2, self.cout)
        self.bwd_ws = ctx.f32(B * (3 * self.cout + max(self.cout // 16, 1)))
        self.dy = None
        self.w = None if self.small else GemmWeight(ctx, conv.weight, "conv3")
        self.bred, self.bred_rows, self.bred_ready = None, 0, False

    def bstat_slab(self, rows_total: int, per_image: bool):
        B = self.x.B
        if per_image and rows_total % B:
            return None
        rows = -(-rows_total // B)
        if self.bred is None or self.bred_rows != rows:
            self.bred, self.bred_rows = self.ctx.f32(B * rows, 2, self.cout), rows
        return self.bred, (self.y, self.scale, self.shift)

    def forward_conv(self, training: bool, sync=None) -> None:
        s = _lib.stream_ptr()
        self.sync = sync if training else None
        if training and self.M <= 1 and not sync:
            raise ValueError("Expected more than 1 value per channel when training, got input size "
                             f"torch.Size([{self.x.B}, {self.cout}, {self.x.H}, {self.x.W}])")
        if self.small:
            w = self.conv.weight.detach()
            call("insar_conv3x3_small_fwd", self.x.ref, ptr(w), self.y.ref, ptr(self.stats) if training else 0, s)
        elif self.c64_fwd:
            self.ctx.join_side()
            _conv3x3_c64(self.x, self.y, self.w.fwd(), 0, self.stats if training else None)
        elif self.c64:
            self.ctx.join_side()
            _igemm(self.x, self.y, self.w.fwd(), self.cout, self.x.H, self.x.W, 1, _TAPS3, 0,
                   stats=self.stats if training else None)
        elif self.flat_fwd:
            self.ctx.join_side()
            _conv3x3_flat(self.x, self.y, self.w.fwd(), 0, self.stats if training else None)
        elif self.rows_fwd:
            self.ctx.join_side()
            _conv3x3_flat(self.x, self.y, self.w.fwd(), 0, self.stats if training else None, geo=self.rows_fwd)
        else:
            self.ctx.join_side()
            _igemm(self.x, self.y, self.w.fwd(), self.cout, self.x.H, self.x.W, 1, _TAPS3, 0,
                   stats=self.stats if training else None)
        if training and self.stat_rps:
            call("insar_colsum_partial", ptr(self.stats), ptr(self.sums), self.stat_rows, 2 * self.cout, self.stat_rps, s)
        part, rows, count = ptr(self.sums), self.fold_rows, self.M
        if self.sync:
            import torch.distributed as dist
            pg, world = self.sync
            if self.sync_sums is None:
                self.sync_sums = self.ctx.f32(2 * self.cout)
            self.ctx.colsum(self.sums, self.sync_sums, 1, self.fold_rows, 2 * self.cout)
            dist.all_reduce(self.sync_sums, op=dist.ReduceOp.SUM, group=pg)
            part, rows, count = ptr(self.sync_sums), 1, self.M * world
        d = bn_finalize_desc(self.bn, part, rows, count, self.cout, training, ptr(self.conv.bias) if self.conv.bias is not None else 0,
                             ptr(self.scale), ptr(self.shift), ptr(self.mean), ptr(self.invstd))
        call("insar_bn_finalize", C.byref(d), s)

    def apply(self, dst: Act, gate: Optional[torch.Tensor], pooled: Optional[Act] = None,
              pool_arg: Optional[torch.Tensor] = None) -> None:
        if pooled is not None and ((self.y.H | self.y.W) & 1):
            call("insar_bn_relu_apply", self.y.ref, ptr(self.scale), ptr(self.shift), ptr(gate), dst.ref, 1, _lib.stream_ptr())
            call("insar_maxpool2_fwd", dst.ref, pooled.ref, _lib.stream_ptr())
            return
        if pooled is not None:
            if pool_arg is not None:
                call("insar_bn_relu_apply_pool_arg", self.y.ref, ptr(self.scale), ptr(self.shift), ptr(gate), dst.ref,
                     pooled.ref, ptr(pool_arg), 1, _lib.stream_ptr())
            else:
                call("insar_bn_relu_apply_pool", self.y.ref, ptr(self.scale), ptr(self.shift), ptr(gate), dst.ref,
                     pooled.ref, 1, _lib.stream_ptr())
            return
        call("insar_bn_relu_apply", self.y.ref, ptr(self.scale), ptr(self.shift), ptr(gate), dst.ref, 1,
             _lib.stream_ptr())

    def _coef(self, coef_args, s, se) -> None:
        if COEF_SIMPLE and se is None:
            call("insar_bn_bwd_coef", coef_args[0], coef_args[1], coef_args[2] * self.x.B, coef_args[3], coef_args[6], coef_args[7], s)
        elif COEF_FUSE and se is None:
            if self._ticket is None:
                self._ticket = torch.zeros(1, dtype=torch.int32, device=self.ctx.device)
            call("insar_bnse_bwd_coef_fused", *coef_args, ptr(self._ticket), s)
        else:
            call("insar_bnse_bwd_coef", *coef_args, s)

    def _sync_k(self) -> None:
        if getattr(self, "sync", None):
            import torch.distributed as dist
            pg, world = self.sync
            if dist.get_backend(pg) == "nccl":
                dist.all_reduce(self.k12, op=dist.ReduceOp.AVG, group=pg)
            else:
                dist.all_reduce(self.k12, op=dist.ReduceOp.SUM, group=pg)
                self.k12.div_(world)

    def backward(self, dout: Optional[Act], sink: GradSink, training: bool, se: Optional["SEState"], dx: Optional[Act],
                 outc_grad=None, pool_grad=None, bstat_for: Optional["ConvBN"] = None, bstat_se: bool = False) -> None:
        ctx, s = self.ctx, _lib.stream_ptr()
        B, H, W = self.x.B, self.x.H, self.x.W
        fuse_small = (self.small and SMALL_WGRAD_FUSE and SMALL_WGRAD_MAIN and dx is None and se is None and outc_grad is None
                      and pool_grad is None and dout is not None and not (training and SPLIT_COEF)
                      and call("insar_conv3x3_small_wgrad_fused_ok", self.x.ref, self.y.ref) == 1
                      and call("insar_conv3x3_small_wgrad_fused_ok", self.x.ref, dout.ref) == 1)
        if self.dy is None and not fuse_small:
            self.dy = Act.alloc(B, H, W, self.cout, ctx.dtype, ctx.device)
        if outc_grad is not None:
            dl, wout, K = outc_grad[:3]
            og_gate, og_wpart = (outc_grad[3], outc_grad[4]) if len(outc_grad) > 3 else (None, None)
            call("insar_bnrelu_bwd_reduce_outc", ptr(dl), ptr(wout), K, self.y.ref, ptr(self.scale), ptr(self.shift),
# ... 297 lines not shown
    def forward(self, training: bool, sync=None) -> None:
        if sync:
            raise _lib.InsarError(f"{self.name}: synchronised BatchNorm (DataParallel(sync_bn=True)) is not supported for "
                                  "SpatialAttention; use sync_bn=False")
        if training and self.M <= 1:
            raise ValueError("Expected more than 1 value per channel when training, got input size "
                             f"torch.Size([{self.x.B}, 1, {self.x.H}, {self.x.W}])")
        s = _lib.stream_ptr()
        d = self._desc()
        d.training = int(training)
        ref = C.byref(d)
        call("insar_sa_compress", ref, s)
        call("insar_sa_conv", ref, 1, s)
        self._finalize(self.conv1, self.bn1, self.stat1, 0, training, s)
        call("insar_sa_conv", ref, 2, s)
        self._finalize(self.conv2, self.bn2, self.stat2, 1, training, s)
        call("insar_sa_gate", ref, s)

    def backward(self, dout: Act, sink: GradSink, training: bool) -> None:
        s = _lib.stream_ptr()
        d = self._desc()
        d.y, d.training = dout.desc, int(training)
        v = lambda p: ptr(sink.view(p))
        d.dw1, d.db1, d.dgamma1, d.dbeta1 = v(self.conv1.weight), v(self.conv1.bias), v(self.bn1.weight), v(self.bn1.bias)
        d.dw2, d.db2, d.dgamma2, d.dbeta2 = v(self.conv2.weight), v(self.conv2.bias), v(self.bn2.weight), v(self.bn2.bias)
        ref = C.byref(d)
        call("insar_sa_dscale", ref, s)
        call("insar_sa_bwd_coef", ref, 2, s)
        call("insar_sa_bwd_stencil", ref, 2, s)
        call("insar_sa_bwd_coef", ref, 1, s)
        call("insar_sa_bwd_stencil", ref, 1, s)
        call("insar_sa_bwd_coef", ref, 0, s)
        call("insar_sa_dx", ref, s)


class UpPlan:

    def __init__(self, ctx: Ctx, mod: torch.nn.ConvTranspose2d, x: Act, out: Act, name: str):
        self.ctx, self.mod, self.x, self.out, self.name = ctx, mod, x, out, name
        self.cin, self.cout = mod.in_channels, mod.out_channels
        if self.cin % 64 or self.cout % 64:
            raise _lib.InsarError(f"{name}: channels must be multiples of 64 on the HIP path")
        self.w = GemmWeight(ctx, mod.weight, "convT")
        self.resize = (out.H, out.W) != (2 * x.H, 2 * x.W)
        if self.resize and not (2 * x.H <= out.H <= 2 * x.H + 1 and 2 * x.W <= out.W <= 2 * x.W + 1):
            raise _lib.InsarError(f"{name}: output {out.H}x{out.W} is not the skip size of a {x.H}x{x.W} input")
        self.conv_out = Act.alloc(x.B, 2 * x.H, 2 * x.W, self.cout, ctx.dtype, ctx.device) if self.resize else out
        self.dconv_out = None
        out_h = self.conv_out.H
        self.bias_rpp = _rows_per_part(out.B, out_h)
        self.bias_rows = out.B * -(-out_h // self.bias_rpp)
        self.bias_part = ctx.f32(self.bias_rows, 2, self.cout)
        self.bias_sum = ctx.f32(2, self.cout)

    def params(self):
        return [self.mod.weight, self.mod.bias]

    def forward(self) -> None:
        self.ctx.join_side()
        _igemm(self.x, self.conv_out, self.w.fwd(), 4 * self.cout, self.x.H, self.x.W, 1, [(0, 0)], 1,
               bias=self.mod.bias.detach() if self.mod.bias is not None else None)
        if self.resize:
            call("insar_resize_bilinear_fwd", self.conv_out.ref, self.out.ref, _lib.stream_ptr())

    def backward(self, dout: Act, sink: GradSink, dx: Optional[Act], consumer: Optional["DoubleConvPlan"] = None) -> None:
        ctx, s = self.ctx, _lib.stream_ptr()
        x, B, h, w = self.x, self.x.B, self.x.H, self.x.W
        if self.resize:
            if self.dconv_out is None:
                co = self.conv_out
                self.dconv_out = Act.alloc(co.B, co.H, co.W, co.c_len, ctx.dtype, ctx.device)
            call("insar_resize_bilinear_bwd", dout.ref, self.dconv_out.ref, s)
            dout = self.dconv_out
        tabx = ctx.pixel_table(B, h, w, 1, h, w, 0)
        tabdy = ctx.pixel_table(B, h, w, 2, dout.H, dout.W, 0)
        mpad = tabx.numel()
        tm, tn = _wgrad_tiles(self.cin, self.cout, ctx.code)
        tiles = 4 * (self.cin // tm) * (self.cout // tn)
        fill = _side_fill(ctx, WGRAD_FILL_T) if (ctx.side is not None and not (PROFILER is not None and PROFILER.alone)) else 1.0
        nsplit = _wgrad_nsplit(tiles, mpad // WG_BKP, 4 * self.cout * self.cin, tm, tn, ctx.esize, fill=fill)
        def weight_grad():
            with ctx.side_stream():
                if self.mod.bias is not None:
                    call("insar_bnrelu_bwd_reduce", dout.ref, dout.ref, ptr(ctx.const(0.0, self.cout)),
                         ptr(ctx.const(1.0, self.cout)), ptr(self.bias_part), 0, self.bias_rpp, _lib.stream_ptr())
                    ctx.colsum(self.bias_part, sink.view(self.mod.bias), 1, self.bias_rows, self.cout, ld=2 * self.cout)
                part = ctx.wgrad_part(nsplit * 4 * self.cout * self.cin)
                d = InsarWgrad()
                d.x, d.dy = x.desc, dout.desc
                d.tabx, d.tabdy, d.part = ptr(tabx), ptr(tabdy), ptr(part)
                d.Mpad, d.nsplit, d.ntaps = mpad, nsplit, 4
                for i, (a, b) in enumerate(_TAPS2):
                    d.offx[i] = 0
                    d.offdy[i] = a * (dout.W + 2) + b
                _launch_wgrad(d, B * h * w, self.cin, self.cout, 4, ctx.code)
                ctx.wgrad_finish(part, sink.view(self.mod.weight), nsplit, 4, self.cout, self.cin, 1)

        if not WGRAD_LATE:
            weight_grad()
        if dx is not None:
            unit = consumer.u2 if (consumer is not None and consumer.pool_arg is None) else None
            slab = _igemm_bstat_slab(unit, consumer is not None and consumer.se is not None, B * h * w, self.cin, h * w, dx)
            _igemm(dout, dx, self.w.dgrad(), self.cin, h, w, 2, _TAPS2, 0,
                   stats=slab[0] if slab else None, bstat=slab[1] if slab else None)
            if slab:
                unit.bred_ready = True
        if WGRAD_LATE:
            weight_grad()


class OutConvPlan:

    def __init__(self, ctx: Ctx, mod: torch.nn.Conv2d, x: Act, name: str = "outc"):
        self.ctx, self.mod, self.x = ctx, mod, x
        self.K, self.cin = mod.out_channels, mod.in_channels
        self.nb = call("insar_conv1x1_out_bwd_blocks", x.B, x.H)
        self.cols = self.K * self.cin + self.K
        self.part = ctx.f32(self.nb, self.cols)
        self.folded = ctx.f32(self.cols)
        self.fused_src = None
        self.part_red, self.reduce_rows = None, 0

    def params(self):
        return [self.mod.weight, self.mod.bias]

    def forward(self, out: Optional[torch.Tensor] = None) -> torch.Tensor:
        self.fused_src = None
        x = self.x
        logits = out if out is not None else torch.empty((x.B, self.K, x.H, x.W), dtype=torch.float32, device=self.ctx.device)
        call("insar_conv1x1_out_fwd", x.ref, ptr(self.mod.weight),
             ptr(self.mod.bias) if self.mod.bias is not None else 0, ptr(logits), self.K, _lib.stream_ptr())
        return logits

    def forward_fused(self, unit: "ConvBN", gate: Optional[torch.Tensor], out: Optional[torch.Tensor] = None) -> torch.Tensor:
        y = unit.y
        logits = out if out is not None else torch.empty((y.B, self.K, y.H, y.W), dtype=torch.float32, device=self.ctx.device)
        call("insar_bn_relu_apply_outc", y.ref, ptr(unit.scale), ptr(unit.shift), ptr(gate), ptr(self.mod.weight),
             ptr(self.mod.bias) if self.mod.bias is not None else 0, ptr(logits), self.K, 1, _lib.stream_ptr())
        self.fused_src = (unit, gate)
        return logits

    def backward(self, dlogits: torch.Tensor, sink: GradSink, dx: Optional[Act]) -> None:
        def fold():
            self.ctx.colsum_into_grads(self.part, self.nb, self._grad_views(sink))

        if dx is None and self.reduce_rows:
            return
        if dx is None:
            if self.ctx.side is not None and not (PROFILER is not None and PROFILER.alone) and dlogits.is_cuda:
                if tape.REC is not None:
                    tape.REC.bad("record_stream on the caller's dlogits")
                if torch.cuda.is_current_stream_capturing():
                    self._keep = dlogits
                else:
                    dlogits.record_stream(self.ctx.side)
            with self.ctx.side_stream():
                if self.fused_src is not None:
                    unit, gate = self.fused_src
                    call("insar_conv1x1_out_wgrad_y", unit.y.ref, ptr(unit.scale), ptr(unit.shift), ptr(gate),
                         ptr(self.mod.weight), ptr(dlogits), self.K, ptr(self.part), _lib.stream_ptr())
                else:
                    call("insar_conv1x1_out_wgrad", self.x.ref, ptr(self.mod.weight), ptr(dlogits), self.K,
                         ptr(self.part), _lib.stream_ptr())
                fold()
            return
        call("insar_conv1x1_out_bwd", self.x.ref, ptr(self.mod.weight), ptr(dlogits), self.K, dx.ref,
             ptr(self.part), _lib.stream_ptr())
        with self.ctx.side_stream():
# ... 65 lines not shown
        sa_mods = [getattr(net, f"sa{i + 1}") for i in range(4)] if getattr(net, "spatial_attention", False) else None
        self.gcat = [A(l, 2 * widths[l]) for l in range(4)] if sa_mods else None

        self.enc: List[DoubleConvPlan] = []
        enc_mods = [net.inc] + [d[1] for d in downs]
        enc_names = ["inc"] + [f"down{i}.1" for i in range(1, 5)]
        for l in range(5):
            xin = self.xin if l == 0 else self.pooled[l - 1]
            out = self.cat[l].slice(0, widths[l]) if l < 4 else self.x5
            self.enc.append(DoubleConvPlan(ctx, enc_mods[l], xin, out, enc_names[l]))
            if l < 4:
                self.enc[l].pool_out = self.pooled[l]
                ch = 16 // ctx.esize
                if POOL_FUSE and widths[l] % ch == 0 and 256 % (widths[l] // ch) == 0 and not ((hs[l] | ws[l]) & 1):
                    self.enc[l].pool_arg = torch.zeros((B, hs[l + 1], ws[l + 1], widths[l]), dtype=torch.uint8, device=device)
        ups = [net.up1, net.up2, net.up3, net.up4]
        convs = [net.conv1, net.conv2, net.conv3, net.conv4]
        self.up: List[UpPlan] = []
        self.dconv: List[DoubleConvPlan] = []
        for i in range(4):
            l = 3 - i
            src = self.x5 if i == 0 else self.dec[l + 1]
            self.up.append(UpPlan(ctx, ups[i], src, self.cat[l].slice(widths[l], widths[l]), f"up{i + 1}"))
            self.dconv.append(DoubleConvPlan(ctx, convs[i], self.gcat[l] if sa_mods else self.cat[l], self.dec[l], f"conv{i + 1}"))
        self.sa: Optional[List[SAUnit]] = ([SAUnit(ctx, sa_mods[i], self.cat[3 - i], self.gcat[3 - i], f"sa{i + 1}") for i in range(4)]
                                           if sa_mods else None)
        self.outc = OutConvPlan(ctx, net.outc, self.dec[0])
        groups = grad_groups(net)
        self.grad_params = [p for g in groups for p in g]
        self.sink = GradSink(ctx, None, groups)
        self.stage_sizes = self.sink.group_sizes
        self.stage_ends = [sum(self.stage_sizes[:i + 1]) for i in range(len(self.stage_sizes))]
        self._gate_events = None
        self.busy = False
        self.training = True
        gws = [b.u1.w for b in self.enc + self.dconv if b.u1.w is not None] + [b.u2.w for b in self.enc + self.dconv]
        gws += [u.w for u in self.up]
        self.weightset = WeightSet(ctx, gws)
        self.bn_modules = [u.bn for b in self.enc + self.dconv for u in (b.u1, b.u2)]
        if self.sa:
            self.bn_modules += [bn for u in self.sa for bn in (u.bn1, u.bn2)]
        self._tape_setup()

    def forward(self, x: torch.Tensor, training: bool) -> torch.Tensor:
        if not (self._tape_allowed(training, not self.net._hooks.get("param_waits")) and self.outc.virtual_grad_ok()):
            return self._forward_eager(x, training)
        if x.dtype != torch.float32 or not x.is_contiguous():
            x = x.float().contiguous()
        logits = torch.empty((self.B, self.outc.K, self.H, self.W), dtype=torch.float32, device=self.ctx.device)
        slots = {"x": x.data_ptr(), "logits": logits.data_ptr()}
        box = {}

        def eager():
            box["out"] = self._forward_eager(x, training)
            return box["out"]

        out, replayed = self._run(self._tape_key("f"), eager, slots, {x.data_ptr(): "x"},
                                  dyn_after=lambda o: {o.data_ptr(): "logits"})
        if replayed:
            self.training = training
            return logits
        return out

    def _stage_gates(self, waits):
        sets = self.weightset.stage_sets(self.sink.groups)
        n = len(self.sink.groups)
        if self._gate_events is None:
            self._gate_events = [torch.cuda.Event() for _ in range(n)]
        with self.ctx.side_stream():
            for st in reversed(range(n)):
                waits(st)
                if sets[st] is not None:
                    sets[st].refresh()
                self._gate_events[st].record()
        self.ctx._side_busy = False
        evs = self._gate_events
        return lambda st: torch.cuda.current_stream().wait_event(evs[st])

    def _forward_eager(self, x: torch.Tensor, training: bool) -> torch.Tensor:
        s = _lib.stream_ptr
        self.training = training
        waits = self.net._hooks.get("param_waits")
        gate = None
        if waits is not None and self.ctx.side is not None:
            gate = self._stage_gates(waits)
        elif PREP_SIDE:
            if waits is not None:
                for st in range(len(self.sink.groups)):
                    waits(st)
            with self.ctx.side_stream():
                self.weightset.refresh()
        else:
            self.weightset.refresh()
        pack_input(x, self.xin)
        sync = self.net._hooks.get("sync_bn") if training else None
        for l in range(5):
            if gate:
                gate(8 - l)
            self.enc[l].forward(training, sync=sync)
        for i in range(3):
            if gate:
                gate(3 - i)
            self.up[i].forward()
            if self.sa:
                self.sa[i].forward(training, sync)
            self.dconv[i].forward(training, sync=sync)
        if gate:
            gate(0)
        self.up[3].forward()
        if self.sa:
            self.sa[3].forward(training, sync)
        if self.outc.virtual_grad_ok():
            return self.dconv[3].forward(training, self.outc, sync=sync)
        self.dconv[3].forward(training, sync=sync)
        return self.outc.forward()

    def backward(self, dlogits: torch.Tensor, on_bucket=None) -> List[torch.Tensor]:
        if dlogits.dtype != torch.float32 or not dlogits.is_contiguous():
            dlogits = dlogits.float().contiguous()
        self.sink.select()
        if not (self._tape_allowed(self.training, on_bucket is None and not self.weightset.stale()) and self.outc.virtual_grad_ok()):
            return self._backward_eager(dlogits, on_bucket)
        out, replayed = self._run(self._tape_key("b"), lambda: self._backward_eager(dlogits, None),
                                  {"dlogits": dlogits.data_ptr()}, {dlogits.data_ptr(): "dlogits"})
        if replayed:
            return [self.sink.view(p) for p in self.grad_params]
        return out

    def _backward_eager(self, dlogits: torch.Tensor, on_bucket=None) -> List[torch.Tensor]:
        s = _lib.stream_ptr
        sink, training, w = self.sink, self.training, self.widths
        fuse = self.outc.virtual_grad_ok()
        wg = self.outc.fused_grad(self.dconv[3].u2) if fuse else None
        self.outc.backward(dlogits, sink, None if fuse else self.ddec[0])
        for i in (3, 2, 1, 0):
            l = 3 - i
            og = (dlogits, self.net.outc.weight.detach(), self.outc.K) if (fuse and i == 3) else None
            if og and wg:
                og = og + wg
            self.dconv[i].backward(None if og else self.ddec[l], sink, training, self.dcat[l], og)
            if og and wg:
                self.outc.fold_fused(sink)
            if self.sa:
                self.sa[i].backward(self.dcat[l], sink, training)
            dsrc = self.dx5 if i == 0 else self.ddec[l + 1]
            self.up[i].backward(self.dcat[l].slice(w[l], w[l]), sink, dsrc, self.enc[4] if i == 0 else self.dconv[i - 1])
            if on_bucket is not None:
                on_bucket(self, ("dec", i))
        for l in (4, 3, 2, 1, 0):
            dout = self.dx5 if l == 4 else self.dcat[l].slice(0, w[l])
            pg = (self.dpooled[l], self.enc[l].pool_arg) if (l < 4 and self.enc[l].pool_arg is not None) else None
            self.enc[l].backward(dout, sink, training, self.dpooled[l - 1] if l > 0 else None, None, pg)
            if l > 0 and self.enc[l - 1].pool_arg is None:
                call("insar_maxpool2_bwd", self.enc[l - 1].out.ref, self.dpooled[l - 1].ref,
                     self.dcat[l - 1].slice(0, w[l - 1]).ref, 1, s())
            if on_bucket is not None:
                on_bucket(self, ("enc", l))
        self.ctx.join_side()
        return [sink.view(p) for p in self.grad_params]
```

### insar_unet_ca_amd/loss.py

```python
from __future__ import annotations

import math
import warnings

import torch
import torch.nn as nn

from . import _lib
from ._lib import call, ptr


def _require_device(logits: torch.Tensor, who: str) -> None:
    if not logits.is_cuda:
        raise _lib.InsarError(f"{who}: logits are on {logits.device}; the HIP path needs a ROCm tensor (no CPU fallback)")


def _prep(logits: torch.Tensor, target: torch.Tensor, who: str):
    _require_device(logits, who)
    if logits.dim() < 2:
        raise _lib.InsarError(f"{who}: logits must be [B, K, ...]")
    B, K = logits.shape[0], logits.shape[1]
    HW = 1
    for d in logits.shape[2:]:
        HW *= d
    if target.shape != (B,) + tuple(logits.shape[2:]):
        raise _lib.InsarError(f"{who}: target shape {tuple(target.shape)} does not match logits {tuple(logits.shape)}")
    lg = logits.detach()
    if lg.dtype != torch.float32 or not lg.is_contiguous():
        lg = lg.float().contiguous()
    tg = target
    if tg.dtype != torch.int64 or not tg.is_contiguous():
        tg = tg.long().contiguous()
    return lg, tg, B, K, HW


def _scale_by(dl: torch.Tensor, g: torch.Tensor, in_dtype) -> torch.Tensor:
    if g.numel() != 1 or not g.is_cuda:
        out = dl * g.detach().to(dl.device, dl.dtype)
        return out if in_dtype == torch.float32 else out.to(in_dtype)
    gs = g.detach()
    if gs.dtype != torch.float32:
        gs = gs.float()
    out = torch.empty_like(dl)
    call("insar_mul_dev_f32", ptr(out), ptr(dl), dl.numel(), ptr(gs), _lib.stream_ptr())
    return out if in_dtype == torch.float32 else out.to(in_dtype)


class _CEFn(torch.autograd.Function):
    @staticmethod
    def forward(ctx, logits, target, ignore_index):
        lg, tg, B, K, HW = _prep(logits, target, "CrossEntropyLoss")
        dl = torch.empty_like(lg)
        nb = call("insar_ce_blocks", B * HW)
        ws = torch.empty(2 + 2 * nb, dtype=torch.float32, device=lg.device)
        out = torch.empty(1, dtype=torch.float32, device=lg.device)
        call("insar_cross_entropy", ptr(lg), ptr(tg), B, K, HW, ignore_index, ptr(dl), ptr(out), ptr(ws), _lib.stream_ptr())
        ctx.dl = dl
        ctx.in_dtype = logits.dtype
        return out[0]

    @staticmethod
    def backward(ctx, g):
        return _scale_by(ctx.dl, g, ctx.in_dtype), None, None


class _DiceFn(torch.autograd.Function):
    @staticmethod
    def forward(ctx, logits, target, ignore_index, smooth):
        lg, tg, B, K, HW = _prep(logits, target, "DiceLoss")
        dl = torch.empty_like(lg)
        nb = call("insar_ce_blocks", B * HW)
        ws = torch.empty(3 * K * (nb + 1), dtype=torch.float32, device=lg.device)
        out = torch.empty(1, dtype=torch.float32, device=lg.device)
        call("insar_dice", ptr(lg), ptr(tg), B, K, HW, ignore_index, float(smooth), ptr(dl), ptr(out), ptr(ws),
             _lib.stream_ptr())
        ctx.dl = dl
        ctx.in_dtype = logits.dtype
        return out[0]

    @staticmethod
    def backward(ctx, g):
        return _scale_by(ctx.dl, g, ctx.in_dtype), None, None, None


class _DiceCEFn(torch.autograd.Function):

    @staticmethod
    def forward(ctx, logits, target, ignore_index, smooth, ce_weight, dice_weight):
        lg, tg, B, K, HW = _prep(logits, target, "DiceCELoss")
        dl = torch.empty_like(lg)
        nb = call("insar_ce_blocks", B * HW)
        ws = torch.empty(3 + 3 * K + nb * (2 + 3 * K), dtype=torch.float32, device=lg.device)
        out = torch.empty(3, dtype=torch.float32, device=lg.device)
        call("insar_dice_ce", ptr(lg), ptr(tg), B, K, HW, ignore_index, float(smooth), float(ce_weight), float(dice_weight),
             ptr(dl), ptr(out), ptr(ws), _lib.stream_ptr())
        ctx.dl = dl
        ctx.in_dtype = logits.dtype
        ctx.parts = out
        return out[0]

    @staticmethod
    def backward(ctx, g):
        return _scale_by(ctx.dl, g, ctx.in_dtype), None, None, None, None, None


class _CEWFn(torch.autograd.Function):

    @staticmethod
    def forward(ctx, logits, target, weight, ignore_index, label_smoothing):
        lg, tg, B, K, HW = _prep(logits, target, "CrossEntropyLoss")
        dl = torch.empty_like(lg)
        nb = call("insar_ce_blocks", B * HW)
        ws = torch.empty(2 + 2 * nb, dtype=torch.float32, device=lg.device)
        out = torch.empty(1, dtype=torch.float32, device=lg.device)
        call("insar_cross_entropy_w", ptr(lg), ptr(tg), B, K, HW, ignore_index, ptr(weight), float(label_smoothing), ptr(dl),
             ptr(out), ptr(ws), _lib.stream_ptr())
        ctx.dl = dl
        ctx.in_dtype = logits.dtype
        return out[0]

    @staticmethod
    def backward(ctx, g):
        return _scale_by(ctx.dl, g, ctx.in_dtype), None, None, None, None


class _FocalFn(torch.autograd.Function):
    @staticmethod
    def forward(ctx, logits, target, alpha, ignore_index, gamma):
        lg, tg, B, K, HW = _prep(logits, target, "FocalLoss")
        dl = torch.empty_like(lg)
        nb = call("insar_ce_blocks", B * HW)
        ws = torch.empty(2 + 2 * nb, dtype=torch.float32, device=lg.device)
        out = torch.empty(1, dtype=torch.float32, device=lg.device)
        call("insar_focal", ptr(lg), ptr(tg), B, K, HW, ignore_index, float(gamma), ptr(alpha), ptr(dl), ptr(out), ptr(ws),
             _lib.stream_ptr())
        ctx.dl = dl
        ctx.in_dtype = logits.dtype
        return out[0]

    @staticmethod
    def backward(ctx, g):
        return _scale_by(ctx.dl, g, ctx.in_dtype), None, None, None, None


class _DiceCEWFn(torch.autograd.Function):

    @staticmethod
    def forward(ctx, logits, target, weight, ignore_index, smooth, ce_weight, dice_weight, label_smoothing, focal_gamma):
        lg, tg, B, K, HW = _prep(logits, target, "DiceCELoss")
        dl = torch.empty_like(lg)
        nb = call("insar_ce_blocks", B * HW)
        ws = torch.empty(4 + 3 * K + nb * (3 + 3 * K), dtype=torch.float32, device=lg.device)
        out = torch.empty(3, dtype=torch.float32, device=lg.device)
        call("insar_dice_ce_w", ptr(lg), ptr(tg), B, K, HW, ignore_index, float(smooth), float(ce_weight), float(dice_weight),
             ptr(weight), float(label_smoothing), float(focal_gamma), ptr(dl), ptr(out), ptr(ws), _lib.stream_ptr())
        ctx.dl = dl
        ctx.in_dtype = logits.dtype
        ctx.parts = out
        return out[0]

    @staticmethod
    def backward(ctx, g):
        return _scale_by(ctx.dl, g, ctx.in_dtype), None, None, None, None, None, None, None, None


MAX_CLASSES = 16


def _class_vector(v, who: str, what: str) -> torch.Tensor:
    t = v.detach().clone() if isinstance(v, torch.Tensor) else torch.as_tensor(v)
    if t.dim() != 1 or t.numel() < 1:
        raise _lib.InsarError(f"{who}: {what} must be a non-empty 1-D vector with one value per class, got shape {tuple(t.shape)}")
    if t.numel() > MAX_CLASSES:
        raise _lib.InsarError(f"{who}: {what} has {t.numel()} classes; the HIP path handles up to {MAX_CLASSES}")
    t = t.to(torch.float32).contiguous()
    if not bool(torch.isfinite(t).all()) or bool((t < 0).any()):
        raise _lib.InsarError(f"{who}: {what} must be finite and non-negative, got {t.tolist()}")
    return t


def _check_smoothing(label_smoothing, who: str) -> float:
    ls = float(label_smoothing)
    if not (0.0 <= ls < 1.0):
        raise _lib.InsarError(f"{who}: label_smoothing={label_smoothing} must be in [0, 1)")
    return ls

# ... 156 lines not shown
```

### insar_unet_ca_amd/tape.py

```python
from __future__ import annotations

import sys
import ctypes as C
import os
from typing import Callable, Dict, List, Optional

import torch

from . import _lib

MODE = os.environ.get("INSAR_TAPE", "1")
REC: Optional["Recorder"] = None


class Recorder:
    def __init__(self, main_ptr: int, side_ptr: int, dyn: Dict[int, str]):
        self.entries: list = []
        self.main_ptr, self.side_ptr, self.dyn = main_ptr, side_ptr, dyn
        self.poison: Optional[str] = None

    def op(self, kind: str, payload=None) -> None:
        self.entries.append((kind, payload))

    def bad(self, why: str) -> None:
# ... 23 lines not shown
            want = self.side_ptr if in_side else self.main_ptr
            if args[-1] != want:
                self.poison = f"{name}: launched on a stream the tape does not model"
                return None
            body = list(args[:-1])
            dyn = [(i, self.dyn[a]) for i, a in enumerate(body) if isinstance(a, int) and a in self.dyn]
            for i, _ in dyn:
                body[i] = 0
            if dyn:
                ops.append((2, fn, body, 1 if in_side else 0, dyn, name))
            else:
                ops.append((1 if in_side else 0, fn, tuple(body), name))
        return ops


def _same_arg(a, b) -> bool:
    if type(a) is not type(b):
        return False
    if isinstance(a, (int, float, bytes, str)) or a is None:
        return a == b
    obj_a, obj_b = getattr(a, "_obj", None), getattr(b, "_obj", None)
    if obj_a is not None and obj_b is not None:
        return bytes(obj_a) == bytes(obj_b)
    if isinstance(a, C.Structure):
        return bytes(a) == bytes(b)
    return a is b


def same_tape(t1: Optional[list], t2: Optional[list]) -> Optional[str]:
    if t1 is None or t2 is None:
        return "a recording could not be turned into a tape"
    if len(t1) != len(t2):
        return f"{len(t1)} vs {len(t2)} ops"
    for i, (a, b) in enumerate(zip(t1, t2)):
        if a[0] != b[0]:
            return f"op {i}: kind {a[0]} vs {b[0]}"
        k = a[0]
        if k in (0, 1):
            if a[1] is not b[1] or len(a[2]) != len(b[2]) or not all(_same_arg(x, y) for x, y in zip(a[2], b[2])):
                return f"op {i} ({a[3]}): arguments differ"
        elif k == 2:
            if a[1] is not b[1] or a[3] != b[3] or a[4] != b[4] or not all(_same_arg(x, y) for x, y in zip(a[2], b[2])):
                return f"op {i} ({a[5]}): arguments differ"
    return None


def tape_py(fn: Callable[[], None]) -> None:
    fn()
    if REC is not None:
        REC.op("py", fn)


def tape_live(fn: Callable[[], None]) -> None:
    global REC
    rec = REC
    if rec is None:
        fn()
        return
    REC, _lib._TAPE = None, None
    try:
        fn()
    finally:
        REC, _lib._TAPE = rec, rec.entries
    rec.op("py", fn)


class PlanTape:

    def _tape_setup(self) -> None:
        self._tapes: Dict[tuple, dict] = {}
        self._tape_params = list(self.net.parameters())
        self._closes: Dict[int, set] = {}

    def bucket_closes(self, min_elems: int) -> set:
        if min_elems not in self._closes:
            from .parallel import plan_buckets
            self._closes[min_elems] = set(plan_buckets(self.stage_sizes, min_elems))
        return self._closes[min_elems]

    def _tape_key(self, which: str) -> tuple:
        from . import engine
        bn = tuple((m.momentum, m.eps) for m in self.bn_modules)
        flags = (engine.BSTAT_FUSE, engine.BSTAT_C64, engine.COEF_SIMPLE, engine.COEF_FUSE, engine.SPLIT_COEF, engine.POOL_FUSE,
                 engine.OUTC_FUSE, engine.OUTC_WGRAD_FUSE, engine.PREP_SIDE, engine.SMALL_WGRAD_MAIN, engine.SMALL_WGRAD_FUSE, engine.WGRAD_LATE, engine.WGRAD_ROWS, engine.WGRAD_X, engine.WGRAD_Y, engine.WGRAD_K, engine.FLAT_PP, engine.FLAT2, engine.FLAT2_KMAX, engine.FLAT2_PERSIST,
                 engine.FLAT_PERSIST, engine.FLAT_ROWS, engine.IGEMM_PP, engine.WGRAD_FILL, engine.WGRAD_FILL_SMALL, engine.WGRAD_FILL_T, engine.WGRAD_FILL_DL, engine.WGRAD_GRID_CAP,
                 getattr(sys.modules.get(__package__ + ".deeplab"), "GATE_FUSE", None), getattr(sys.modules.get(__package__ + ".deeplab"), "GATE_STATS", None))
        return (which, self.sink.active if which == "b" else 0, hash(bn), hash(flags))

    def _tape_fingerprint(self) -> int:
        ptrs = [p.data_ptr() for p in self._tape_params]
        for m in self.bn_modules:
            ptrs.append(m.running_mean.data_ptr() if m.running_mean is not None else 0)
            ptrs.append(m.running_var.data_ptr() if m.running_var is not None else 0)
            ptrs.append(m.num_batches_tracked.data_ptr() if m.num_batches_tracked is not None else 0)
        return hash(tuple(ptrs))

    def _tape_allowed(self, training: bool, extra_ok: bool = True) -> bool:
        from . import engine
        return (MODE != "0" and training and extra_ok and engine.PROFILER is None and self.ctx.side is not None
                and not self.net._hooks.get("sync_bn") and not torch.cuda.is_current_stream_capturing())

    def _run(self, key: tuple, eager: Callable, slots: Dict[str, int], dyn_ptrs: Dict[int, str], dyn_after=None):
        st = self._tapes.setdefault(key, {"state": 0, "tape": None, "calls": 0, "fp": None})
        st["calls"] += 1
        fp = self._tape_fingerprint()
        if st["fp"] != fp:
            if st["state"] not in (0, -1):
                st["moved"] = st.get("moved", 0) + 1
            st["state"], st["tape"], st["fp"] = (0 if st.get("moved", 0) < 8 else -1), None, fp
        if st["state"] == 3:
            if MODE == "verify" and st["calls"] % 16 == 0:
                out, rec = self._record(eager, dyn_ptrs, dyn_after)
                why = same_tape(st["tape"], rec)
                if why:
                    raise _lib.InsarError(f"launch tape {key}: the live launch sequence departed from the tape: {why}")
                return out, False
            self._replay(st["tape"], slots)
            return None, True
        if st["state"] in (0, -1):
            if st["state"] == 0:
                st["state"] = 1
            return eager(), False
        out, rec = self._record(eager, dyn_ptrs, dyn_after)
        if st["state"] == 1:
            st["tape"], st["state"] = rec, 2
        else:
            why = same_tape(st["tape"], rec)
            st["state"] = 3 if why is None else -1
            st["why"] = why
            if why is not None:
                st["tape"] = None
        return out, False

    def _record(self, eager: Callable, dyn_ptrs: Dict[int, str], dyn_after=None):
        global REC
        side = self.ctx.side.cuda_stream
        rec = Recorder(_lib.stream_ptr(), side, dict(dyn_ptrs))
        REC, _lib._TAPE = rec, rec.entries
        try:
            out = eager()
        finally:
            REC, _lib._TAPE = None, None
        if dyn_after is not None:
            rec.dyn.update(dyn_after(out))
        return out, rec.finish()

    def _replay(self, ops: list, slots: Dict[str, int]) -> None:
        ctx = self.ctx
        main = _lib.stream_ptr()
        side = ctx.side.cuda_stream
        prev = None
        try:
            for op in ops:
                k = op[0]
                if k == 0:
                    rc = op[1](*op[2], main)
                elif k == 1:
                    rc = op[1](*op[2], side)
                elif k == 2:
                    body = list(op[2])
                    for i, slot in op[4]:
                        body[i] = slots[slot]
                    rc = op[1](*body, side if op[3] else main)
                elif k == 3:
                    prev = ctx._side_enter()
                    continue
                elif k == 4:
# ... 20 lines not shown
```

Baseline: 2336 tiles/s.

## Add direct NCHW first conv, late loss grad, and plain row-sum bias reduce

Three separate changes. A first-conv variant reads the fp32 NCHW input directly and converts it to bf16 inside the MFMA kernel, which lets input packing move to the side stream. A dice+CE option defers the gradient kernel to backward and scales it by the upstream gradient on device. The conv bias gradient now uses a dedicated row-sum kernel instead of the bnrelu reduce with identity scale and shift. The first two are off by default (env flags set to "0"), so only the row-sum bias reduction runs by default; it avoids reading y and the affine arithmetic for a small side-stream reduction.

After: 2337 tiles/s, median of 6. Within noise of the previous version (+0.0%).

```diff
diff --git a/include/insar_hip.h b/include/insar_hip.h
--- a/include/insar_hip.h
+++ b/include/insar_hip.h
@@ -133,6 +133,8 @@
 int insar_conv3x3_small_fwd_rows(const InsarAct* x, const InsarAct* y);
 int insar_conv3x3_small_fwd(const InsarAct* x, const float* w ,
                             const InsarAct* y, float* stats , void* stream);
+int insar_conv3x3_small_fwd_nchw(const float* src, const InsarAct* x, const float* w, const InsarAct* y,
+                                 float* stats, void* stream);
 int insar_conv3x3_small_wgrad_blocks(int32_t B, int32_t H);
 int insar_conv3x3_small_wgrad(const InsarAct* x, const InsarAct* dy, float* part, void* stream);
 int insar_conv3x3_small_wgrad_fused_ok(const InsarAct* x, const InsarAct* y);
@@ -296,6 +298,9 @@
 int insar_dice_ce(const float* logits, const int64_t* target, int32_t B, int32_t K, int64_t HW,
                   int64_t ignore_index, float smooth, float ce_weight, float dice_weight, float* dlogits,
                   float* loss_out, float* ws, void* stream);
+int insar_dice_ce_grad(const float* logits, const int64_t* target, int32_t B, int32_t K, int64_t HW,
+                       int64_t ignore_index, float smooth, float ce_weight, float dice_weight, const float* ws,
+                       const float* upstream, float* dlogits, void* stream);
 
 int insar_cross_entropy_w(const float* logits, const int64_t* target, int32_t B, int32_t K, int64_t HW,
                           int64_t ignore_index, const float* weight, float label_smoothing, float* dlogits,
diff --git a/insar_unet_ca_amd/_lib.py b/insar_unet_ca_amd/_lib.py
--- a/insar_unet_ca_amd/_lib.py
+++ b/insar_unet_ca_amd/_lib.py
@@ -147,6 +147,7 @@
     "insar_wgrad_fold": [_P, _P, _L, _I, _I, _P],
     "insar_pixel_table": [_P, _L, _I, _I, _I, _I, _I, _I, _I, _P],
     "insar_conv3x3_small_fwd": [_AP, _P, _AP, _P, _P],
+    "insar_conv3x3_small_fwd_nchw": [_P, _AP, _P, _AP, _P, _P],
     "insar_conv3x3_small_fwd_rows": [_AP, _AP],
     "insar_conv3x3_small_wgrad_blocks": [_I, _I],
     "insar_conv3x3_small_wgrad": [_AP, _AP, _P, _P],
@@ -197,6 +198,7 @@
     "insar_cross_entropy": [_P, _P, _I, _I, _L, _L, _P, _P, _P, _P],
     "insar_dice": [_P, _P, _I, _I, _L, _L, _F, _P, _P, _P, _P],
     "insar_dice_ce": [_P, _P, _I, _I, _L, _L, _F, _F, _F, _P, _P, _P, _P],
+    "insar_dice_ce_grad": [_P, _P, _I, _I, _L, _L, _F, _F, _F, _P, _P, _P, _P],
     "insar_confusion": [_P, _P, _I, _I, _L, _L, _P, _P],
     "insar_cross_entropy_w": [_P, _P, _I, _I, _L, _L, _P, _F, _P, _P, _P, _P],
     "insar_focal": [_P, _P, _I, _I, _L, _L, _F, _P, _P, _P, _P, _P],
diff --git a/insar_unet_ca_amd/csrc/direct.hip b/insar_unet_ca_amd/csrc/direct.hip
--- a/insar_unet_ca_amd/csrc/direct.hip
+++ b/insar_unet_ca_amd/csrc/direct.hip
@@ -101,9 +101,10 @@
 typedef __attribute__((ext_vector_type(8))) short d_bf16x8_t;
 typedef __attribute__((ext_vector_type(4))) float d_f32x4_t;
 
-template <int CI>
+template <int CI, bool NCHW = false>
 __global__ void __launch_bounds__(DR_THREADS) conv3x3_small_fwd_mfma_kernel(ActView x, const float* __restrict__ wt, ActView y,
-                                                                           float* __restrict__ part) {
+                                                                           float* __restrict__ part,
+                                                                           const float* __restrict__ src = nullptr) {
   constexpr int KV = 9 * CI;
   __shared__ float red[DR_THREADS / 64][2][64];
   const int lane = threadIdx.x & 63, wave = threadIdx.x >> 6, nw = blockDim.x >> 6;
@@ -136,7 +137,20 @@
       const int wc = ok ? w : y.W - 1;
       d_bf16x8_t xf;
       const char* p0 = x.base + x.elem_offset(n, h - 1, wc - 1) * (int64_t)sizeof(bf16_t);
-      if constexpr (CI == 2) {
+      if constexpr (NCHW) {
+#pragma unroll
+        for (int i = 0; i < 8; ++i) {
+          const int k = 8 * kq + i;
+          short v = 0;
+          if (k < KV) {
+            const int tap = k / CI, ci = k - tap * CI;
+            const int hh = h - 1 + tap / 3, ww = wc - 1 + tap % 3;
+            if ((unsigned)hh < (unsigned)x.H && (unsigned)ww < (unsigned)x.W)
+              v = (short)f32_to_bf16(src[(((int64_t)n * CI + ci) * x.H + hh) * x.W + ww]);
+          }
+          xf[i] = v;
+        }
+      } else if constexpr (CI == 2) {
 #pragma unroll
         for (int i = 0; i < 4; ++i) {
           const int tap = 4 * kq + i;
@@ -245,9 +259,9 @@
   if (small_fwd_uses_mfma(x, y)) {
     grid = insar_conv3x3_small_fwd_rows(x, y);
     switch (x->c_len) {
-      case 1: hipLaunchKernelGGL((conv3x3_small_fwd_mfma_kernel<1>), dim3(grid), dim3(DR_THREADS), 0, s, xv, w, yv, stats); break;
-      case 2: hipLaunchKernelGGL((conv3x3_small_fwd_mfma_kernel<2>), dim3(grid), dim3(DR_THREADS), 0, s, xv, w, yv, stats); break;
-      default: hipLaunchKernelGGL((conv3x3_small_fwd_mfma_kernel<3>), dim3(grid), dim3(DR_THREADS), 0, s, xv, w, yv, stats); break;
+      case 1: hipLaunchKernelGGL((conv3x3_small_fwd_mfma_kernel<1>), dim3(grid), dim3(DR_THREADS), 0, s, xv, w, yv, stats, (const float*)nullptr); break;
+      case 2: hipLaunchKernelGGL((conv3x3_small_fwd_mfma_kernel<2>), dim3(grid), dim3(DR_THREADS), 0, s, xv, w, yv, stats, (const float*)nullptr); break;
+      default: hipLaunchKernelGGL((conv3x3_small_fwd_mfma_kernel<3>), dim3(grid), dim3(DR_THREADS), 0, s, xv, w, yv, stats, (const float*)nullptr); break;
     }
   } else if (y->dtype == INSAR_BF16) {
     switch (x->c_len) { case 1: SMALL_FWD(bf16_t, 1); break; case 2: SMALL_FWD(bf16_t, 2); break;
@@ -258,6 +272,24 @@
   }
 #undef SMALL_FWD
   INSAR_CHECK_LAUNCH("insar_conv3x3_small_fwd");
+  return INSAR_OK;
+}
+
+extern "C" int insar_conv3x3_small_fwd_nchw(const float* src, const InsarAct* x, const float* w, const InsarAct* y, float* stats,
+                                            void* stream) {
+  int rc;
+  if ((rc = check_small(x, y, "insar_conv3x3_small_fwd_nchw"))) return rc;
+  if (!src || !w) INSAR_FAIL(INSAR_E_ARG, "insar_conv3x3_small_fwd_nchw: null pointer");
+  if (!small_fwd_uses_mfma(x, y)) INSAR_FAIL(INSAR_E_SHAPE, "insar_conv3x3_small_fwd_nchw: bf16, Cin <= 3, Cout = 64 only");
+  const int grid = insar_conv3x3_small_fwd_rows(x, y);
+  hipStream_t s = (hipStream_t)stream;
+  const ActView xv = make_view(*x), yv = make_view(*y);
+  switch (x->c_len) {
+    case 1: hipLaunchKernelGGL((conv3x3_small_fwd_mfma_kernel<1, true>), dim3(grid), dim3(DR_THREADS), 0, s, xv, w, yv, stats, src); break;
+    case 2: hipLaunchKernelGGL((conv3x3_small_fwd_mfma_kernel<2, true>), dim3(grid), dim3(DR_THREADS), 0, s, xv, w, yv, stats, src); break;
+    default: hipLaunchKernelGGL((conv3x3_small_fwd_mfma_kernel<3, true>), dim3(grid), dim3(DR_THREADS), 0, s, xv, w, yv, stats, src); break;
+  }
+  INSAR_CHECK_LAUNCH("insar_conv3x3_small_fwd_nchw");
   return INSAR_OK;
 }
 
diff --git a/insar_unet_ca_amd/csrc/loss_optim.hip b/insar_unet_ca_amd/csrc/loss_optim.hip
--- a/insar_unet_ca_amd/csrc/loss_optim.hip
+++ b/insar_unet_ca_amd/csrc/loss_optim.hip
@@ -330,9 +330,11 @@
 template <int KT>
 __global__ void dicece_grad_v4(const float* __restrict__ logits, const int64_t* __restrict__ target, int64_t HW,
                                int64_t npix, int64_t ignore_index, float smooth, float ce_w, float dice_w,
-                               const float* __restrict__ ws, float* __restrict__ dlogits) {
+                               const float* __restrict__ ws, const float* __restrict__ gup, float* __restrict__ dlogits) {
   float num[KT], den[KT];
   const float inv = ws[1] * ce_w;
+  const bool scaled = gup != nullptr;
+  const float g = scaled ? gup[0] : 1.f;
 #pragma unroll
   for (int k = 0; k < KT; ++k) {
     num[k] = 2.f * ws[3 + k] + smooth;
@@ -370,7 +372,10 @@
           dot = fmaf(pr[k], gk[k], dot);
         }
 #pragma unroll
-        for (int k = 0; k < KT; ++k) o[k] = (pr[k] - (k == t ? 1.f : 0.f)) * inv + dice_w * pr[k] * (gk[k] - dot);
+        for (int k = 0; k < KT; ++k) {
+          o[k] = (pr[k] - (k == t ? 1.f : 0.f)) * inv + dice_w * pr[k] * (gk[k] - dot);
+          if (scaled) o[k] *= g;
+        }
       }
 #pragma unroll
       for (int k = 0; k < KT; ++k) ((float*)&gv[k])[e] = o[k];
@@ -382,9 +387,11 @@
 
 __global__ void dicece_grad_kernel(const float* __restrict__ logits, const int64_t* __restrict__ target, int K, int64_t HW,
                                    int64_t npix, int64_t ignore_index, float smooth, float ce_w, float dice_w,
-                                   const float* __restrict__ ws, float* __restrict__ dlogits) {
+                                   const float* __restrict__ ws, const float* __restrict__ gup, float* __restrict__ dlogits) {
   float num[LO_MAXK], den[LO_MAXK];
   const float inv = ws[1] * ce_w;
+  const bool scaled = gup != nullptr;
+  const float g = scaled ? gup[0] : 1.f;
 #pragma unroll
   for (int k = 0; k < LO_MAXK; ++k) {
     num[k] = k < K ? 2.f * ws[3 + k] + smooth : 0.f;
@@ -413,38 +420,65 @@
     }
 #pragma unroll
     for (int k = 0; k < LO_MAXK; ++k)
-      if (k < K) gp[k * HW] = (pr[k] - (k == t ? 1.f : 0.f)) * inv + dice_w * pr[k] * (gk[k] - dot);
-  }
+      if (k < K) {
+        float o = (pr[k] - (k == t ? 1.f : 0.f)) * inv + dice_w * pr[k] * (gk[k] - dot);
+        if (scaled) o *= g;
+        gp[k * HW] = o;
+      }
+  }
+}
+
+static bool dicece_v4_ok(int32_t K, int64_t HW, const float* logits, const int64_t* target, const float* dlogits) {
+  return K >= 2 && K <= 4 && (HW & 3) == 0 && insar_aligned16(logits) && insar_aligned16(target) && (!dlogits || insar_aligned16(dlogits));
+}
+
+static void dicece_launch_grad(const float* logits, const int64_t* target, int32_t K, int64_t HW, int64_t npix, int nb,
+                               int64_t ignore_index, float smooth, float ce_weight, float dice_weight, const float* ws,
+                               const float* gup, float* dlogits, hipStream_t s) {
+#define DICECE_G4(KT)                                                                                                        \
+  hipLaunchKernelGGL(dicece_grad_v4<KT>, dim3(nb), dim3(LO_THREADS), 0, s, logits, target, HW, npix, ignore_index, smooth, \
+                     ce_weight, dice_weight, ws, gup, dlogits)
+  const bool v4 = dicece_v4_ok(K, HW, logits, target, dlogits);
+  if (v4 && K == 2) DICECE_G4(2);
+  else if (v4 && K == 3) DICECE_G4(3);
+  else if (v4 && K == 4) DICECE_G4(4);
+  else
+    hipLaunchKernelGGL(dicece_grad_kernel, dim3(nb), dim3(LO_THREADS), 0, s, logits, target, K, HW, npix, ignore_index, smooth,
+                       ce_weight, dice_weight, ws, gup, dlogits);
+#undef DICECE_G4
 }
 
 extern "C" int insar_dice_ce(const float* logits, const int64_t* target, int32_t B, int32_t K, int64_t HW, int64_t ignore_index,
                              float smooth, float ce_weight, float dice_weight, float* dlogits, float* loss_out, float* ws,
                              void* stream) {
-  if (!logits || !target || !dlogits || !loss_out || !ws) INSAR_FAIL(INSAR_E_ARG, "insar_dice_ce: null pointer");
+  if (!logits || !target || !loss_out || !ws) INSAR_FAIL(INSAR_E_ARG, "insar_dice_ce: null pointer");
   if (K < 1 || K > LO_MAXK) INSAR_FAIL(INSAR_E_SHAPE, "insar_dice_ce: num_classes=%d must be 1..%d", K, LO_MAXK);
   if (B < 1 || HW < 1) INSAR_FAIL(INSAR_E_SHAPE, "insar_dice_ce: bad shape");
   const int64_t npix = (int64_t)B * HW;
   const int nb = insar_ce_blocks(npix);
   hipStream_t s = (hipStream_t)stream;
-  const bool v4 = K >= 2 && K <= 4 && (HW & 3) == 0 && insar_aligned16(logits) && insar_aligned16(target) && insar_aligned16(dlogits);
-#define DICECE_V4(KT)                                                                                                              \
-  do {                                                                                                                             \
-    hipLaunchKernelGGL(dicece_partial_v4<KT>, dim3(nb), dim3(LO_THREADS), 0, s, logits, target, HW, npix, ignore_index, ws);        \
-    hipLaunchKernelGGL(dicece_final_kernel, dim3(1), dim3(LO_THREADS), 0, s, ws, K, nb, smooth, ce_weight, dice_weight, loss_out); \
-    hipLaunchKernelGGL(dicece_grad_v4<KT>, dim3(nb), dim3(LO_THREADS), 0, s, logits, target, HW, npix, ignore_index, smooth,        \
-                       ce_weight, dice_weight, ws, dlogits);                                                                        \
-  } while (0)
-  if (v4 && K == 2) DICECE_V4(2);
-  else if (v4 && K == 3) DICECE_V4(3);
-  else if (v4 && K == 4) DICECE_V4(4);
-  else {
-    hipLaunchKernelGGL(dicece_partial_kernel, dim3(nb), dim3(LO_THREADS), 0, s, logits, target, K, HW, npix, ignore_index, ws);
-    hipLaunchKernelGGL(dicece_final_kernel, dim3(1), dim3(LO_THREADS), 0, s, ws, K, nb, smooth, ce_weight, dice_weight, loss_out);
-    hipLaunchKernelGGL(dicece_grad_kernel, dim3(nb), dim3(LO_THREADS), 0, s, logits, target, K, HW, npix, ignore_index, smooth,
-                       ce_weight, dice_weight, ws, dlogits);
-  }
-#undef DICECE_V4
+  const bool v4 = dicece_v4_ok(K, HW, logits, target, dlogits);
+  if (v4 && K == 2) hipLaunchKernelGGL(dicece_partial_v4<2>, dim3(nb), dim3(LO_THREADS), 0, s, logits, target, HW, npix, ignore_index, ws);
+  else if (v4 && K == 3) hipLaunchKernelGGL(dicece_partial_v4<3>, dim3(nb), dim3(LO_THREADS), 0, s, logits, target, HW, npix, ignore_index, ws);
+  else if (v4 && K == 4) hipLaunchKernelGGL(dicece_partial_v4<4>, dim3(nb), dim3(LO_THREADS), 0, s, logits, target, HW, npix, ignore_index, ws);
+  else hipLaunchKernelGGL(dicece_partial_kernel, dim3(nb), dim3(LO_THREADS), 0, s, logits, target, K, HW, npix, ignore_index, ws);
+  hipLaunchKernelGGL(dicece_final_kernel, dim3(1), dim3(LO_THREADS), 0, s, ws, K, nb, smooth, ce_weight, dice_weight, loss_out);
+  if (dlogits)
+    dicece_launch_grad(logits, target, K, HW, npix, nb, ignore_index, smooth, ce_weight, dice_weight, ws, nullptr, dlogits, s);
   INSAR_CHECK_LAUNCH("insar_dice_ce");
+  return INSAR_OK;
+}
+
+extern "C" int insar_dice_ce_grad(const float* logits, const int64_t* target, int32_t B, int32_t K, int64_t HW,
+                                  int64_t ignore_index, float smooth, float ce_weight, float dice_weight, const float* ws,
+                                  const float* upstream, float* dlogits, void* stream) {
+  if (!logits || !target || !ws || !dlogits) INSAR_FAIL(INSAR_E_ARG, "insar_dice_ce_grad: null pointer");
+  if (K < 1 || K > LO_MAXK) INSAR_FAIL(INSAR_E_SHAPE, "insar_dice_ce_grad: num_classes=%d must be 1..%d", K, LO_MAXK);
+  if (B < 1 || HW < 1) INSAR_FAIL(INSAR_E_SHAPE, "insar_dice_ce_grad: bad shape");
+  const int64_t npix = (int64_t)B * HW;
+  dicece_launch_grad(logits, target, K, HW, npix, insar_ce_blocks(npix), ignore_index, smooth, ce_weight, dice_weight, ws,
+                     upstream, dlogits, (hipStream_t)stream);
+  INSAR_CHECK_LAUNCH("insar_dice_ce_grad");
   return INSAR_OK;
 }
 
diff --git a/insar_unet_ca_amd/csrc/pointwise.hip b/insar_unet_ca_amd/csrc/pointwise.hip
--- a/insar_unet_ca_amd/csrc/pointwise.hip
+++ b/insar_unet_ca_amd/csrc/pointwise.hip
@@ -938,8 +938,84 @@
   return INSAR_OK;
 }
 
+template <typename T>
+__global__ void __launch_bounds__(1024) row_sum_kernel(ActView g, float* __restrict__ part, int rpp) {
+  constexpr int CH = Chunk<T>::N;
+  __shared__ float red[PW_THREADS][CH + 1];
+  const int cpp = g.c_len / CH;
+  const int ppi = (g.H + rpp - 1) / rpp;
+  const int nparts = g.B * ppi;
+  const bool inv = (blockDim.x % cpp) == 0;
+  for (int r = blockIdx.x; r < nparts; r += gridDim.x) {
+    const int n = r / ppi, h0 = (r - n * ppi) * rpp;
+    const int h1 = min(g.H, h0 + rpp);
+    if (inv) {
+      float a0[CH];
+      const int cc = threadIdx.x % cpp;
+#pragma unroll
+      for (int j = 0; j < CH; ++j) a0[j] = 0.f;
+      const int wstep = blockDim.x / cpp;
+      for (int h = h0; h < h1; ++h) {
+        for (int w0 = threadIdx.x / cpp; w0 < g.W; w0 += PW_UNROLL * wstep) {
+          uint4 vg[PW_UNROLL];
+#pragma unroll
+          for (int u = 0; u < PW_UNROLL; ++u)
+            if (w0 + u * wstep < g.W) vg[u] = *chunk_ptr<T>(g, n, h, w0 + u * wstep, cc);
+#pragma unroll
+          for (int u = 0; u < PW_UNROLL; ++u)
+            if (w0 + u * wstep < g.W) {
+              float gg[CH];
+              Chunk<T>::unpack(vg[u], gg);
+#pragma unroll
+              for (int j = 0; j < CH; ++j) a0[j] += gg[j];
+            }
+        }
+      }
+#pragma unroll
+      for (int j = 0; j < CH; ++j) red[threadIdx.x][j] = a0[j];
+      __syncthreads();
+      for (int c = threadIdx.x; c < g.c_len; c += blockDim.x) {
+        const int occ = c / CH, j = c - occ * CH;
+        float s = 0.f;
+        for (int t = occ; t < blockDim.x; t += cpp) s += red[t][j];
+        part[(int64_t)r * 2 * g.c_len + c] = s;
+      }
+      __syncthreads();
+    } else {
+      for (int c = threadIdx.x; c < g.c_len; c += blockDim.x) {
+        float s0 = 0.f;
+        for (int h = h0; h < h1; ++h)
+          for (int w = 0; w < g.W; ++w) {
+            const T* pg = (const T*)(g.base + (g.elem_offset(n, h, w) + c) * (int64_t)sizeof(T));
+            if constexpr (sizeof(T) == 2) s0 += bf16_to_f32(*(const uint16_t*)pg); else s0 += *(const float*)pg;
+          }
+        part[(int64_t)r * 2 * g.c_len + c] = s0;
+      }
+    }
+  }
+}
+
+static int launch_row_sum(const char* who, const InsarAct* g, float* part, int32_t rows_per_part, void* stream) {
+  int rc;
+  if ((rc = insar_check_act(g, who, "dout"))) return rc;
+  if (!part) INSAR_FAIL(INSAR_E_ARG, "%s: null pointer", who);
+  if (rows_per_part < 1) INSAR_FAIL(INSAR_E_SHAPE, "%s: rows_per_part", who);
+  if (g->c_len % (g->dtype == INSAR_BF16 ? 8 : 4)) INSAR_FAIL(INSAR_E_SHAPE, "%s: C=%d is not a whole number of 16-byte chunks", who, g->c_len);
+  const int rpp = rows_per_part;
+  const int grid = insar_grid_cap((int64_t)g->B * ((g->H + rpp - 1) / rpp));
+  const ActView v = make_view(*g);
+  if (g->dtype == INSAR_BF16) hipLaunchKernelGGL(row_sum_kernel<bf16_t>, dim3(grid), dim3(PW_THREADS), 0, (hipStream_t)stream, v, part, rpp);
+  else hipLaunchKernelGGL(row_sum_kernel<float>, dim3(grid), dim3(PW_THREADS), 0, (hipStream_t)stream, v, part, rpp);
+  INSAR_CHECK_LAUNCH(who);
+  return INSAR_OK;
+}
+
 extern "C" int insar_bnrelu_bwd_reduce(const InsarAct* dout, const InsarAct* y, const float* scale, const float* shift,
                                        float* part, int32_t relu, int32_t rows_per_part, void* stream) {
+  if (!scale && !shift) {
+    if (relu) INSAR_FAIL(INSAR_E_ARG, "insar_bnrelu_bwd_reduce: relu needs scale and shift");
+    return launch_row_sum("insar_bnrelu_bwd_reduce", dout, part, rows_per_part, stream);
+  }
   return launch_bwd_reduce("insar_bnrelu_bwd_reduce", dout, y, scale, shift, part, relu, rows_per_part,
                            OutcGrad{nullptr, nullptr, 0, nullptr, nullptr}, PoolGrad{ActView{}, nullptr}, stream);
 }
diff --git a/insar_unet_ca_amd/engine.py b/insar_unet_ca_amd/engine.py
--- a/insar_unet_ca_amd/engine.py
+++ b/insar_unet_ca_amd/engine.py
@@ -299,6 +299,8 @@
 POOL_FUSE = os.environ.get("INSAR_POOL_FUSE", "1") != "0"
 SMALL_WGRAD_FUSE = os.environ.get("INSAR_SMALL_WGRAD_FUSE", "1") != "0"
 SMALL_WGRAD_MAIN = os.environ.get("INSAR_SMALL_WGRAD_MAIN", "1") != "0"
+FIRST_DIRECT = os.environ.get("INSAR_FIRST_DIRECT", "0") != "0"
+BIAS_ROW_SUM = os.environ.get("INSAR_BIAS_ROW_SUM", "1") != "0"
 PREP_SIDE = os.environ.get("INSAR_PREP_SIDE", "1") != "0"
 OUTC_FUSE = os.environ.get("INSAR_OUTC_FUSE", "1") != "0"
 WGRAD_GRID_CAP = int(os.environ.get("INSAR_WGRAD_GRID_CAP", "200"))
@@ -581,6 +583,7 @@
             raise _lib.InsarError(f"{name}: input slice has {x.c_len} channels, conv expects {self.cin}")
         self.small = self.cin <= 4
         self._small_part = None
+        self.direct_src = None
         if not self.small and self.cin % 64:
             raise _lib.InsarError(f"{name}: in_channels={self.cin} must be <=4 or a multiple of 64 on the HIP path")
         if self.cout % 64:
@@ -643,7 +646,11 @@
                              f"torch.Size([{self.x.B}, {self.cout}, {self.x.H}, {self.x.W}])")
         if self.small:
             w = self.conv.weight.detach()
-            call("insar_conv3x3_small_fwd", self.x.ref, ptr(w), self.y.ref, ptr(self.stats) if training else 0, s)
+            if self.direct_src is not None:
+                call("insar_conv3x3_small_fwd_nchw", ptr(self.direct_src), self.x.ref, ptr(w), self.y.ref,
+                     ptr(self.stats) if training else 0, s)
+            else:
+                call("insar_conv3x3_small_fwd", self.x.ref, ptr(w), self.y.ref, ptr(self.stats) if training else 0, s)
         elif self.c64_fwd:
             self.ctx.join_side()
             _conv3x3_c64(self.x, self.y, self.w.fwd(), 0, self.stats if training else None)
@@ -1107,8 +1114,12 @@
         def weight_grad():
             with ctx.side_stream():
                 if self.mod.bias is not None:
-                    call("insar_bnrelu_bwd_reduce", dout.ref, dout.ref, ptr(ctx.const(0.0, self.cout)),
-                         ptr(ctx.const(1.0, self.cout)), ptr(self.bias_part), 0, self.bias_rpp, _lib.stream_ptr())
+                    if BIAS_ROW_SUM:
+                        call("insar_bnrelu_bwd_reduce", dout.ref, dout.ref, 0, 0, ptr(self.bias_part), 0, self.bias_rpp,
+                             _lib.stream_ptr())
+                    else:
+                        call("insar_bnrelu_bwd_reduce", dout.ref, dout.ref, ptr(ctx.const(0.0, self.cout)),
+                             ptr(ctx.const(1.0, self.cout)), ptr(self.bias_part), 0, self.bias_rpp, _lib.stream_ptr())
                     ctx.colsum(self.bias_part, sink.view(self.mod.bias), 1, self.bias_rows, self.cout, ld=2 * self.cout)
                 part = ctx.wgrad_part(nsplit * 4 * self.cout * self.cin)
                 d = InsarWgrad()
@@ -1340,6 +1351,12 @@
         self.training = training
         waits = self.net._hooks.get("param_waits")
         gate = None
+        u0 = self.enc[0].u1
+        direct = (FIRST_DIRECT and PREP_SIDE and training and waits is None and self.ctx.side is not None and u0.small
+                  and u0.cin <= 3 and u0.cout == 64 and self.ctx.dtype == torch.bfloat16)
+        if direct and (x.dtype != torch.float32 or not x.is_contiguous()):
+            x = x.float().contiguous()
+        u0.direct_src = x if direct else None
         if waits is not None and self.ctx.side is not None:
             gate = self._stage_gates(waits)
         elif PREP_SIDE:
@@ -1348,9 +1365,12 @@
                     waits(st)
             with self.ctx.side_stream():
                 self.weightset.refresh()
+                if direct:
+                    pack_input(x, self.xin)
         else:
             self.weightset.refresh()
-        pack_input(x, self.xin)
+        if not direct:
+            pack_input(x, self.xin)
         sync = self.net._hooks.get("sync_bn") if training else None
         for l in range(5):
             if gate:
diff --git a/insar_unet_ca_amd/loss.py b/insar_unet_ca_amd/loss.py
--- a/insar_unet_ca_amd/loss.py
+++ b/insar_unet_ca_amd/loss.py
@@ -1,6 +1,7 @@
 from __future__ import annotations
 
 import math
+import os
 import warnings
 
 import torch
@@ -8,6 +9,9 @@
 
 from . import _lib
 from ._lib import call, ptr
+
+
+LATE_GRAD = os.environ.get("INSAR_LOSS_LATE_GRAD", "0") != "0"
 
 
 def _require_device(logits: torch.Tensor, who: str) -> None:
@@ -88,20 +92,35 @@
     @staticmethod
     def forward(ctx, logits, target, ignore_index, smooth, ce_weight, dice_weight):
         lg, tg, B, K, HW = _prep(logits, target, "DiceCELoss")
-        dl = torch.empty_like(lg)
+        late = LATE_GRAD
+        dl = None if late else torch.empty_like(lg)
         nb = call("insar_ce_blocks", B * HW)
         ws = torch.empty(3 + 3 * K + nb * (2 + 3 * K), dtype=torch.float32, device=lg.device)
         out = torch.empty(3, dtype=torch.float32, device=lg.device)
         call("insar_dice_ce", ptr(lg), ptr(tg), B, K, HW, ignore_index, float(smooth), float(ce_weight), float(dice_weight),
              ptr(dl), ptr(out), ptr(ws), _lib.stream_ptr())
         ctx.dl = dl
+        if late:
+            ctx.save_for_backward(lg, tg)
+            ctx.ws, ctx.geom = ws, (B, K, HW, ignore_index, float(smooth), float(ce_weight), float(dice_weight))
         ctx.in_dtype = logits.dtype
         ctx.parts = out
         return out[0]
 
     @staticmethod
     def backward(ctx, g):
-        return _scale_by(ctx.dl, g, ctx.in_dtype), None, None, None, None, None
+        if ctx.dl is not None:
+            return _scale_by(ctx.dl, g, ctx.in_dtype), None, None, None, None, None
+        lg, tg = ctx.saved_tensors
+        dev = g.numel() == 1 and g.is_cuda
+        gs = g.detach() if dev else None
+        if dev and gs.dtype != torch.float32:
+            gs = gs.float()
+        dl = torch.empty_like(lg)
+        call("insar_dice_ce_grad", ptr(lg), ptr(tg), *ctx.geom, ptr(ctx.ws), ptr(gs), ptr(dl), _lib.stream_ptr())
+        if not dev:
+            return _scale_by(dl, g, ctx.in_dtype), None, None, None, None, None
+        return (dl if ctx.in_dtype == torch.float32 else dl.to(ctx.in_dtype)), None, None, None, None, None
 
 
 class _CEWFn(torch.autograd.Function):
diff --git a/insar_unet_ca_amd/tape.py b/insar_unet_ca_amd/tape.py
--- a/insar_unet_ca_amd/tape.py
+++ b/insar_unet_ca_amd/tape.py
@@ -129,7 +129,7 @@
         from . import engine
         bn = tuple((m.momentum, m.eps) for m in self.bn_modules)
         flags = (engine.BSTAT_FUSE, engine.BSTAT_C64, engine.COEF_SIMPLE, engine.COEF_FUSE, engine.SPLIT_COEF, engine.POOL_FUSE,
-                 engine.OUTC_FUSE, engine.OUTC_WGRAD_FUSE, engine.PREP_SIDE, engine.SMALL_WGRAD_MAIN, engine.SMALL_WGRAD_FUSE, engine.WGRAD_LATE, engine.WGRAD_ROWS, engine.WGRAD_X, engine.WGRAD_Y, engine.WGRAD_K, engine.FLAT_PP, engine.FLAT2, engine.FLAT2_KMAX, engine.FLAT2_PERSIST,
+                 engine.OUTC_FUSE, engine.OUTC_WGRAD_FUSE, engine.PREP_SIDE, engine.FIRST_DIRECT, engine.BIAS_ROW_SUM, engine.SMALL_WGRAD_MAIN, engine.SMALL_WGRAD_FUSE, engine.WGRAD_LATE, engine.WGRAD_ROWS, engine.WGRAD_X, engine.WGRAD_Y, engine.WGRAD_K, engine.FLAT_PP, engine.FLAT2, engine.FLAT2_KMAX, engine.FLAT2_PERSIST,
                  engine.FLAT_PERSIST, engine.FLAT_ROWS, engine.IGEMM_PP, engine.WGRAD_FILL, engine.WGRAD_FILL_SMALL, engine.WGRAD_FILL_T, engine.WGRAD_FILL_DL, engine.WGRAD_GRID_CAP,
                  getattr(sys.modules.get(__package__ + ".deeplab"), "GATE_FUSE", None), getattr(sys.modules.get(__package__ + ".deeplab"), "GATE_STATS", None))
         return (which, self.sink.active if which == "b" else 0, hash(bn), hash(flags))
```
